# gsalzer/mythril

Measured on AMD Instinct MI355X. Metric: constraint-candidate evals/sec + % z3 queries discharged on-GPU, higher is better.
Workload: dtype u32 (256-bit as 8x32-bit limbs)

## Files before the change

mythril_amd/csrc/u256.h:

```cpp
#pragma once
#include <math.h>
#include <stdint.h>

#define PF_INL __device__ __forceinline__

#include "u256_cols.h"

namespace pf {

struct u256 {
    uint32_t l[8];
};

PF_INL u256 zero256() {
    u256 r;
#pragma unroll
    for (int i = 0; i < 8; i++) r.l[i] = 0;
    return r;
}

PF_INL u256 ones256() {
    u256 r;
#pragma unroll
    for (int i = 0; i < 8; i++) r.l[i] = 0xffffffffu;
    return r;
}

PF_INL u256 add256(const u256& a, const u256& b) {
    u256 r;
    uint32_t c = 0;
#pragma unroll
    for (int i = 0; i < 8; i++) {
        uint32_t co;
        r.l[i] = __builtin_addc(a.l[i], b.l[i], c, &co);
        c = co;
    }
    return r;
}

PF_INL u256 add256c(const u256& a, const u256& b, uint32_t* cout) {
    u256 r;
    uint32_t c = 0;
#pragma unroll
    for (int i = 0; i < 8; i++) {
        uint32_t co;
        r.l[i] = __builtin_addc(a.l[i], b.l[i], c, &co);
        c = co;
    }
    *cout = c;
    return r;
}

PF_INL u256 sub256(const u256& a, const u256& b) {
    u256 r;
    uint32_t c = 0;
#pragma unroll
    for (int i = 0; i < 8; i++) {
        uint32_t co;
        r.l[i] = __builtin_subc(a.l[i], b.l[i], c, &co);
        c = co;
    }
    return r;
}

PF_INL u256 sub256b(const u256& a, const u256& b, uint32_t* bout) {
    u256 r;
    uint32_t c = 0;
#pragma unroll
    for (int i = 0; i < 8; i++) {
        uint32_t co;
        r.l[i] = __builtin_subc(a.l[i], b.l[i], c, &co);
        c = co;
    }
    *bout = c;
    return r;
}

PF_INL uint32_t ult256(const u256& a, const u256& b) {
    uint32_t c = 0;
#pragma unroll
    for (int i = 0; i < 8; i++) {
        uint32_t co;
        (void)__builtin_subc(a.l[i], b.l[i], c, &co);
        c = co;
    }
    return c;
}

PF_INL uint32_t eq256(const u256& a, const u256& b) {
    uint32_t d = 0;
#pragma unroll
    for (int i = 0; i < 8; i++) d |= a.l[i] ^ b.l[i];
    return d == 0;
}

PF_INL uint32_t iszero256(const u256& a) {
    uint32_t d = 0;
#pragma unroll
    for (int i = 0; i < 8; i++) d |= a.l[i];
    return d == 0;
}

PF_INL u256 neg256(const u256& a) { return sub256(zero256(), a); }

PF_INL u256 not256(const u256& a) {
    u256 r;
#pragma unroll
    for (int i = 0; i < 8; i++) r.l[i] = ~a.l[i];
    return r;
}

PF_INL uint32_t lane_mask(uint32_t c) {
    uint32_t m = 0u - (uint32_t)(c != 0u);
#ifndef PF_HOST_MAC
    asm volatile("" : "+v"(m));
#endif
    return m;
}

PF_INL uint32_t zero_limb() {
    uint32_t z = 0u;
#ifndef PF_HOST_MAC
    asm("" : "+v"(z));
#endif
    return z;
}

PF_INL u256 sel256(uint32_t c, const u256& a, const u256& b) {
    const uint32_t m = lane_mask(c);
    u256 r;
#pragma unroll
    for (int i = 0; i < 8; i++) r.l[i] = (a.l[i] & m) | (b.l[i] & ~m);
    return r;
}

#ifndef PF_HOST_MAC
PF_INL uint32_t wave_max_u32(uint32_t v) {
#pragma unroll
    for (int o = 32; o >= 1; o >>= 1) v = max(v, (uint32_t)__shfl_xor((int)v, o));
    return __builtin_amdgcn_readfirstlane(v);
}
PF_INL uint64_t wave_mask(bool p) { return __builtin_amdgcn_ballot_w64(p); }
#else
PF_INL uint32_t wave_max_u32(uint32_t v) { return v; }
PF_INL uint64_t wave_mask(bool p) { return p ? 1ull : 0ull; }
#endif
PF_INL bool wave_any(uint64_t m) { return m != 0ull; }
PF_INL bool wave_none(uint64_t m) { return m == 0ull; }

PF_INL uint64_t wave_mask_ult256(const u256& a, const u256& b) {
#ifndef PF_HOST_MAC
    uint64_t m;
    uint32_t t;
    asm("v_sub_co_u32 %1, vcc, %2, %10\n\ts_nop 1\n\t"
        "v_subb_co_u32 %1, vcc, %3, %11, vcc\n\ts_nop 1\n\t"
        "v_subb_co_u32 %1, vcc, %4, %12, vcc\n\ts_nop 1\n\t"
        "v_subb_co_u32 %1, vcc, %5, %13, vcc\n\ts_nop 1\n\t"
        "v_subb_co_u32 %1, vcc, %6, %14, vcc\n\ts_nop 1\n\t"
        "v_subb_co_u32 %1, vcc, %7, %15, vcc\n\ts_nop 1\n\t"
        "v_subb_co_u32 %1, vcc, %8, %16, vcc\n\ts_nop 1\n\t"
        "v_subb_co_u32 %1, %0, %9, %17, vcc"
        : "=s"(m), "=&v"(t)
        : "v"(a.l[0]), "v"(a.l[1]), "v"(a.l[2]), "v"(a.l[3]), "v"(a.l[4]), "v"(a.l[5]), "v"(a.l[6]),
          "v"(a.l[7]), "v"(b.l[0]), "v"(b.l[1]), "v"(b.l[2]), "v"(b.l[3]), "v"(b.l[4]), "v"(b.l[5]),
          "v"(b.l[6]), "v"(b.l[7])
        : "vcc");
    return m;
#else
    return wave_mask(ult256(a, b) != 0u);
#endif
}

PF_INL uint32_t sat_u32(double x) {
#ifndef PF_HOST_MAC
    uint32_t r;
    asm("v_cvt_u32_f64 %0, %1" : "=v"(r) : "v"(x));
    return r;
#else
    return (uint32_t)fmin(x, 4294967295.0);
#endif
}

#define PF_COL_NEXT(k)                                   \
    r.l[k] = (uint32_t)acc;                              \
    acc = (acc >> 32) | ((uint64_t)hi << 32);            \
    hi = 0u;

PF_INL u256 mul256(const u256& a, const u256& b) {
    const uint32_t *x = a.l, *y = b.l;
    u256 r;
    uint64_t acc = 0;
    uint32_t hi = 0;
    col64_1(acc, x[0], y[0]);
    PF_COL_NEXT(0)
    col96_2(acc, hi, x[0], x[1], y[1], y[0]);
    PF_COL_NEXT(1)
    col96_3(acc, hi, x[0], x[1], x[2], y[2], y[1], y[0]);
    PF_COL_NEXT(2)
    col96_4(acc, hi, x[0], x[1], x[2], x[3], y[3], y[2], y[1], y[0]);
    PF_COL_NEXT(3)
    col96_5(acc, hi, x[0], x[1], x[2], x[3], x[4], y[4], y[3], y[2], y[1], y[0]);
    PF_COL_NEXT(4)
    col96_6(acc, hi, x[0], x[1], x[2], x[3], x[4], x[5], y[5], y[4], y[3], y[2], y[1], y[0]);
    PF_COL_NEXT(5)
    col64_7(acc, x[0], x[1], x[2], x[3], x[4], x[5], x[6], y[6], y[5], y[4], y[3], y[2], y[1], y[0]);
    r.l[6] = (uint32_t)acc;
    acc >>= 32;
    col64_8(acc, x[0], x[1], x[2], x[3], x[4], x[5], x[6], x[7], y[7], y[6], y[5], y[4], y[3], y[2], y[1], y[0]);
    r.l[7] = (uint32_t)acc;
    return r;
}

PF_INL u256 sqr256(const u256& a) {
    const uint32_t* x = a.l;
    u256 r;
    r.l[0] = 0u;
    uint64_t acc = 0;
    uint32_t hi = 0;
    col64_1(acc, x[0], x[1]);
    PF_COL_NEXT(1)
    col96_1(acc, hi, x[0], x[2]);
    PF_COL_NEXT(2)
    col96_2(acc, hi, x[0], x[1], x[3], x[2]);
    PF_COL_NEXT(3)
    col96_2(acc, hi, x[0], x[1], x[4], x[3]);
    PF_COL_NEXT(4)
    col96_3(acc, hi, x[0], x[1], x[2], x[5], x[4], x[3]);
    PF_COL_NEXT(5)
    col64_3(acc, x[0], x[1], x[2], x[6], x[5], x[4]);
    r.l[6] = (uint32_t)acc;
    acc >>= 32;
    col64_4(acc, x[0], x[1], x[2], x[3], x[7], x[6], x[5], x[4]);
    r.l[7] = (uint32_t)acc;
    u256 c;
#pragma unroll
    for (int i = 7; i >= 1; i--) c.l[i] = (r.l[i] << 1) | (r.l[i - 1] >> 31);
    c.l[0] = 0u;
    u256 d;
#pragma unroll
    for (int i = 0; i < 4; i++) {
        uint64_t q = 0;
        col64_1(q, x[i], x[i]);
        d.l[2 * i] = (uint32_t)q;
        d.l[2 * i + 1] = (uint32_t)(q >> 32);
    }
    return add256(c, d);
}
#undef PF_COL_NEXT

PF_INL uint32_t mul256_overflows(const u256& a, const u256& b) {
    uint32_t hi = 0;
    u256 r = zero256();
#pragma unroll
    for (int i = 0; i < 8; i++) {
        uint64_t carry = 0;
#pragma unroll
        for (int j = 0; j < 8; j++) {
            if (i + j < 8) {
                uint64_t t = (uint64_t)a.l[i] * b.l[j] + r.l[i + j] + carry;
                r.l[i + j] = (uint32_t)t;
                carry = t >> 32;
            } else {
                hi |= (a.l[i] != 0u && b.l[j] != 0u) ? 1u : 0u;
            }
        }
        hi |= (carry != 0) ? 1u : 0u;
    }
    return hi;
}

PF_INL u256 shl256(const u256& a, uint32_t s, uint32_t big) {
    u256 x = a;
    if (__builtin_expect(1, 1)) {
        uint32_t m = (s >> 7) & 1;
#pragma unroll
        for (int i = 7; i >= 0; i--) x.l[i] = m ? (i >= 4 ? x.l[i - 4] : 0u) : x.l[i];
        m = (s >> 6) & 1;
#pragma unroll
        for (int i = 7; i >= 0; i--) x.l[i] = m ? (i >= 2 ? x.l[i - 2] : 0u) : x.l[i];
        m = (s >> 5) & 1;
#pragma unroll
        for (int i = 7; i >= 0; i--) x.l[i] = m ? (i >= 1 ? x.l[i - 1] : 0u) : x.l[i];
    }
    uint32_t bs = s & 31;
    u256 r;
#pragma unroll
    for (int i = 7; i >= 1; i--) r.l[i] = bs ? ((x.l[i] << bs) | (x.l[i - 1] >> (32 - bs))) : x.l[i];
    r.l[0] = x.l[0] << bs;
    return sel256(big, zero256(), r);
}

PF_INL u256 shr256(const u256& a, uint32_t s, uint32_t f) {
    u256 x = a;
    uint32_t m = (s >> 7) & 1;
#pragma unroll
    for (int i = 0; i < 8; i++) x.l[i] = m ? (i + 4 < 8 ? x.l[i + 4] : f) : x.l[i];
    m = (s >> 6) & 1;
#pragma unroll
    for (int i = 0; i < 8; i++) x.l[i] = m ? (i + 2 < 8 ? x.l[i + 2] : f) : x.l[i];
    m = (s >> 5) & 1;
#pragma unroll
    for (int i = 0; i < 8; i++) x.l[i] = m ? (i + 1 < 8 ? x.l[i + 1] : f) : x.l[i];
    uint32_t bs = s & 31;
    u256 r;
#pragma unroll
    for (int i = 0; i < 7; i++) r.l[i] = bs ? ((x.l[i] >> bs) | (x.l[i + 1] << (32 - bs))) : x.l[i];
    r.l[7] = bs ? ((x.l[7] >> bs) | (f << (32 - bs))) : x.l[7];
    return r;
}

PF_INL uint32_t clz256(const u256& a) {
    uint32_t n = 0, done = 0;
#pragma unroll
    for (int i = 7; i >= 0; i--) {
        uint32_t z = a.l[i] ? (uint32_t)__builtin_clz(a.l[i]) : 32u;
        n += done ? 0u : z;
        done |= (a.l[i] != 0u);
    }
    return n;
}

PF_INL double rcp_f64(double x) {
#ifndef PF_HOST_MAC
    double r = __builtin_amdgcn_rcp(x);
    double e = fma(-x, r, 1.0);
    r = fma(r, e, r);
    e = fma(-x, r, 1.0);
    return fma(r, e, r);
#else
    return 1.0 / x;
#endif
}

PF_INL double to_f64(const u256& a) {
    double d = 0.0;
#pragma unroll
    for (int i = 7; i >= 0; i--) d = fma(d, 4294967296.0, (double)a.l[i]);
    return d;
}

#define PF_DIV_BIAS 0x1p-12
PF_INL void udivrem256(const u256& a, const u256& b, u256* q, u256* r) {
    const uint32_t bz = iszero256(b);
    const uint64_t m_bz = wave_mask(bz != 0u);
#ifndef PF_DIV_FORCE_GENERAL
    if (wave_none(wave_mask(true) & ~(wave_mask_ult256(a, b) | m_bz))) {
        *q = sel256(bz, ones256(), zero256());
        *r = a;
        return;
    }
    if (wave_none(wave_mask((b.l[1] | b.l[2] | b.l[3] | b.l[4] | b.l[5] | b.l[6] | b.l[7]) != 0u))) {
        const uint32_t d = bz ? 1u : b.l[0];
        const double rd = rcp_f64((double)d);
        uint32_t rem = 0;
        u256 Q;
#pragma unroll
        for (int j = 7; j >= 0; j--) {
            const uint64_t num = ((uint64_t)rem << 32) | a.l[j];
            const double dn = (double)rem * 4294967296.0 + (double)a.l[j];
            uint32_t qj = sat_u32(fma(dn, rd, 0x1p-12));
            int64_t rr = (int64_t)(num - (uint64_t)qj * d);
            const uint32_t lo = (uint32_t)(rr < 0);
            qj -= lo;
            rr += (int64_t)(d & lane_mask(lo));
            Q.l[j] = qj;
            rem = (uint32_t)rr;
        }
        u256 R = zero256();
        R.l[0] = rem;
        *q = sel256(bz, ones256(), Q);
        *r = sel256(bz, a, R);
        return;
    }
#endif
    const double rcp = rcp_f64(fmax(to_f64(b), 1.0));
#ifndef PF_DIV_FORCE_GENERAL
    const double qest = fma(to_f64(a), rcp, PF_DIV_BIAS);
    if (wave_none(wave_mask(qest >= 4294967294.0) & ~m_bz)) {
        uint32_t qh = sat_u32(qest);
        u256 R, Q = zero256();
        uint32_t carry = 0, bw = 0;
#pragma unroll
        for (int i = 0; i < 8; i++) {
            const uint64_t p = (uint64_t)qh * b.l[i] + carry;
            carry = (uint32_t)(p >> 32);
            uint32_t bo;
            R.l[i] = __builtin_subc(a.l[i], (uint32_t)p, bw, &bo);
            bw = bo;
        }
        uint32_t bo8;
        const uint32_t r8 = __builtin_subc(zero_limb(), carry, bw, &bo8);
        if (wave_any(wave_mask(r8 != 0u))) {
            const uint32_t neg = (uint32_t)(r8 != 0u);
            const uint32_t m = lane_mask(neg);
            uint32_t c = 0;
#pragma unroll
            for (int i = 0; i < 8; i++) {
                uint32_t co;
                R.l[i] = __builtin_addc(R.l[i], b.l[i] & m, c, &co);
                c = co;
            }
            qh -= neg;
        }
        Q.l[0] = qh;
        *q = sel256(bz, ones256(), Q);
        *r = R;
        return;
    }
#endif
    uint32_t u[9];
#pragma unroll
    for (int i = 0; i < 8; i++) u[i] = a.l[i];
    u256 Q = zero256();
    u[8] = zero_limb();
    uint32_t sfx[9];
    sfx[8] = 0u;
#pragma unroll
    for (int k = 7; k >= 0; k--) sfx[k] = sfx[k + 1] | b.l[k];
#pragma unroll
    for (int j = 7; j >= 0; j--) {
        const uint32_t bhigh = j >= 2 ? sfx[9 - j] : 0u;
        double dr = (double)u[7];
#pragma unroll
        for (int i = 6; i >= j; i--) dr = fma(dr, 4294967296.0, (double)u[i]);
        const double qe = fma(dr, rcp, PF_DIV_BIAS);
        if (wave_none(wave_mask(qe >= 1.0) & ~(m_bz | wave_mask(bhigh != 0u)))) continue;
        const uint32_t skip = bz | (uint32_t)(bhigh != 0u);
        uint32_t q = sat_u32(qe) & ~lane_mask(skip);
        uint64_t carry = 0;
        uint32_t borrow = 0;
#pragma unroll
        for (int i = 0; i + j <= 8; i++) {
            const uint64_t p = (uint64_t)q * (i < 8 ? b.l[i] : 0u) + carry;
            carry = p >> 32;
            uint32_t bo;
            u[j + i] = __builtin_subc(u[j + i], (uint32_t)p, borrow, &bo);
            borrow = bo;
        }
        if (wave_any(wave_mask(u[8] != 0u))) {
            const uint32_t neg = (uint32_t)(u[8] != 0u);
            const uint32_t m = 0u - neg;
            q -= neg;
            uint32_t c = 0;
#pragma unroll
            for (int i = 0; i + j <= 8; i++) {
                uint32_t co;
                u[j + i] = __builtin_addc(u[j + i], (i < 8 ? b.l[i] : 0u) & m, c, &co);
                c = co;
            }
        }
        Q.l[j] = q;
    }
    u256 R;
#pragma unroll
    for (int i = 0; i < 8; i++) R.l[i] = u[i];
    *q = sel256(bz, ones256(), Q);
    *r = R;
}

PF_INL void tbl_put(uint2* tbl, uint32_t stride, uint32_t j, const u256& v) {
#pragma unroll
    for (int p = 0; p < 4; p++) tbl[(j * 4u + p) * stride] = make_uint2(v.l[2 * p], v.l[2 * p + 1]);
}
PF_INL u256 tbl_get(const uint2* tbl, uint32_t stride, uint32_t j) {
    u256 v;
#pragma unroll
    for (int p = 0; p < 4; p++) {
        const uint2 q = tbl[(j * 4u + p) * stride];
        v.l[2 * p] = q.x;
        v.l[2 * p + 1] = q.y;
    }
    return v;
}

template <int WB = 3>
PF_INL u256 exp256(const u256& base, const u256& e, uint32_t nbits, uint2* tbl, uint32_t stride) {
    static_assert(WB >= 1 && WB <= 3, "window");
    constexpr uint32_t NT = 1u << WB;
    u256 r = zero256();
    r.l[0] = 1u;
    if (nbits == 0u) return r;
    tbl_put(tbl, stride, 0u, r);
    tbl_put(tbl, stride, 1u, base);
    if constexpr (WB == 2) {
        const u256 b2 = sqr256(base);
        tbl_put(tbl, stride, 2u, b2);
        tbl_put(tbl, stride, 3u, mul256(b2, base));
    } else {
#pragma unroll 1
        for (uint32_t j = 2; j < NT; j++) {
            const u256 f = tbl_get(tbl, stride, (j & 1u) ? j - 1u : j >> 1);
            const u256 g = (j & 1u) ? base : f;
            tbl_put(tbl, stride, j, mul256(f, g));
        }
    }
    const uint32_t nd = (nbits + WB - 1u) / WB;
    const uint32_t rest = WB * (nd - 1u);
    r = tbl_get(tbl, stride, shr256(e, rest, 0u).l[0] & (NT - 1u));
    u256 ex = shl256(e, (256u - rest) & 255u, 0u);
#pragma unroll 1
    for (uint32_t i = 1; i < nd; i++) {
#pragma unroll 1
        for (int k = 0; k < WB; k++) r = sqr256(r);
        const uint32_t d = ex.l[7] >> (32 - WB);
#pragma unroll
        for (int k = 7; k >= 1; k--) ex.l[k] = (ex.l[k] << WB) | (ex.l[k - 1] >> (32 - WB));
        ex.l[0] <<= WB;
        r = mul256(r, tbl_get(tbl, stride, d));
    }
    return r;
}

template <int WB = 2>
PF_INL u256 exp256_w32(const u256& base, uint32_t e, uint32_t nbits, uint2* tbl, uint32_t stride) {
    static_assert(WB == 2, "window");
    u256 one = zero256();
    one.l[0] = 1u;
    tbl_put(tbl, stride, 1u, base);
    const u256 b2 = sqr256(base);
    tbl_put(tbl, stride, 2u, b2);
    tbl_put(tbl, stride, 3u, mul256(b2, base));
    if (nbits == 0u) return one;
    const uint32_t nd = (nbits + WB - 1u) / WB;
    uint32_t d = (e >> (WB * (nd - 1u))) & 3u;
    u256 r = sel256((uint32_t)(d == 0u), one, tbl_get(tbl, stride, d));
#pragma unroll 1
    for (uint32_t i = nd - 1u; i-- > 0u;) {
#pragma unroll 1
        for (int k = 0; k < WB; k++) r = sqr256(r);
        d = (e >> (WB * i)) & 3u;
        r = mul256(r, sel256((uint32_t)(d == 0u), one, tbl_get(tbl, stride, d)));
    }
    return r;
}

#ifndef PF_EXP_SPLIT
#define PF_EXP_SPLIT 8
#endif
#define PF_EXP_WINDOW (PF_EXP_SPLIT <= 20 ? 2 : 3)
#define PF_EXP_TBL_ENTRIES (1 << PF_EXP_WINDOW)

PF_INL uint32_t funnel(uint32_t hi, uint32_t lo, uint32_t s) {
    return (uint32_t)((((uint64_t)hi << 32) | lo) >> s);
}

template <int L>
PF_INL void tsqr(const uint32_t* a, uint32_t* out) {
    uint32_t r[L];
#pragma unroll
    for (int i = 0; i < L; i++) r[i] = 0u;
#pragma unroll
    for (int i = 0; 2 * i + 1 < L; i++) {
        uint64_t c = 0;
#pragma unroll
        for (int j = i + 1; i + j < L; j++) {
            c = (uint64_t)a[i] * a[j] + (uint64_t)r[i + j] + (c >> 32);
            r[i + j] = (uint32_t)c;
        }
    }
#pragma unroll
    for (int i = L - 1; i >= 1; i--) r[i] = funnel(r[i], r[i - 1], 31u);
    r[0] <<= 1;
    uint32_t d[L];
#pragma unroll
    for (int i = 0; 2 * i < L; i++) {
        const uint64_t q = (uint64_t)a[i] * a[i];
        d[2 * i] = (uint32_t)q;
        if (2 * i + 1 < L) d[2 * i + 1] = (uint32_t)(q >> 32);
    }
    uint32_t c = 0;
#pragma unroll
    for (int i = 0; i < L; i++) {
        uint32_t co;
        out[i] = __builtin_addc(r[i], d[i], c, &co);
        c = co;
    }
}

template <int TL, uint32_t TM, int Q>
PF_INL void t_steps(uint32_t* t, uint32_t k0, uint32_t k1) {
    constexpr int L = TL - Q;
#pragma unroll 1
    for (uint32_t k = k0; k < k1; k++) {
        uint32_t sq[L];
        if constexpr (L == 8) {
            u256 a;
#pragma unroll
            for (int i = 0; i < 8; i++) a.l[i] = t[i];
            const u256 s = sqr256(a);
#pragma unroll
            for (int i = 0; i < 8; i++) sq[i] = s.l[i];
        } else {
            tsqr<L>(t, sq);
        }
        const uint32_t sh = 32u - (k + 1u - 32u * Q);
        uint32_t c = 0;
#pragma unroll
        for (int i = Q; i < TL; i++) {
            const uint32_t lo = i > Q ? sq[i > Q ? i - Q - 1 : 0] : 0u;
            uint32_t co;
            t[i] = __builtin_addc(t[i], funnel(sq[i - Q], lo, sh), c, &co);
            c = co;
        }
        t[TL - 1] &= TM;
    }
}


constexpr int v2c(int i) { return (i & 1) ? 0 : 1 + v2c(i >> 1); }
constexpr int v2fact(int j) { return j <= 1 ? 0 : v2c(j) + v2fact(j - 1); }
constexpr int exp_terms(int m) {
    int j = 1;
    while ((j + 1) * (m + 2) - v2fact(j + 1) < 256) j++;
    return j;
}
constexpr int prefix_val(int m, int i) { return (i - 1) * (m + 2) - v2fact(i - 1); }

struct k256 {
    uint32_t l[8];
};
constexpr k256 k_small(uint32_t v) {
    k256 r{};
    r.l[0] = v;
    return r;
}
constexpr k256 k_mul(const k256& a, const k256& b) {
    k256 r{};
    for (int i = 0; i < 8; i++) {
        uint64_t c = 0;
        for (int j = 0; i + j < 8; j++) {
            c = (uint64_t)a.l[i] * b.l[j] + r.l[i + j] + (c >> 32);
            r.l[i + j] = (uint32_t)c;
        }
    }
    return r;
}
constexpr k256 k_inv(const k256& o) {
    k256 x = o;
    for (int it = 0; it < 7; it++) {
        const k256 ox = k_mul(o, x);
        k256 two_minus{};
        uint64_t bw = 0;
        for (int i = 0; i < 8; i++) {
            const uint64_t d = (uint64_t)(i == 0 ? 2u : 0u) - ox.l[i] - bw;
            two_minus.l[i] = (uint32_t)d;
            bw = (d >> 32) & 1u;
        }
        x = k_mul(x, two_minus);
    }
    return x;
}
constexpr k256 exp_oddprod(int i, int j) {
    k256 r = k_small(1u);
    for (int k = i; k <= j; k++) r = k_mul(r, k_small((uint32_t)(k >> v2c(k))));
    return r;
}
constexpr k256 exp_addend(int i, int j, int limbs) {
    k256 r = k_mul(exp_oddprod(i, j), k_inv(exp_oddprod(1, j)));
    for (int k = limbs; k < 8; k++) r.l[k] = 0u;
    return r;
}

template <int L, int LY, uint32_t K0, uint32_t K1>
PF_INL u256 tmul_add(const u256& a, const u256& b, const k256& k) {
    if constexpr (L >= 8) {
        u256 kk;
#pragma unroll
        for (int i = 0; i < 8; i++) kk.l[i] = k.l[i];
        return add256(mul256(a, b), kk);
    } else {
        u256 r = zero256();
        tmulk<L, LY, K0, K1>(a.l, b.l, k.l, r.l);
        return r;
    }
}

template <int L>
PF_INL u256 tmul(const u256& a, const u256& b) {
    if constexpr (L >= 8)
        return mul256(a, b);
    else
        return tmul_add<L, L, 0u, 0u>(a, b, k256{});
}

template <int L>
PF_INL u256 sub_mul_small(const u256& a, const u256& b, uint32_t c) {
    u256 r = zero256();
    uint32_t carry = 0, bw = 0;
#pragma unroll
    for (int i = 0; i < L; i++) {
        const uint64_t p = (uint64_t)b.l[i] * c + carry;
        carry = (uint32_t)(p >> 32);
        uint32_t bo;
        r.l[i] = __builtin_subc(a.l[i], (uint32_t)p, bw, &bo);
        bw = bo;
    }
    return r;
}

template <int S, int L>
PF_INL u256 shl_const(const u256& a) {
    constexpr int LS = S / 32, BS = S % 32;
    u256 r = zero256();
#pragma unroll
    for (int i = LS; i < L; i++) {
        const uint32_t hi = a.l[i - LS];
        const uint32_t lo = i - LS - 1 >= 0 ? a.l[i - LS - 1 >= 0 ? i - LS - 1 : 0] : 0u;
        r.l[i] = BS ? funnel(hi, lo, 32 - BS) : hi;
    }
    return r;
}

template <int M, int I, int J>
PF_INL u256 horner(u256& g, const u256& tt) {
    constexpr int S = M + 2 - v2c(I);
    constexpr int P = 256 - prefix_val(M, I);
    constexpr int L = (P + 31) / 32;
    constexpr k256 K = exp_addend(I, J, L);
    constexpr int LY = (I == J || (P - S + 31) / 32 >= L || L == 1) ? L : L - 1;
    u256 inner = zero256();
    if constexpr (I < J) {
        inner = horner<M, I + 1, J>(g, tt);
        g = add256(g, tt);
    } else {
        constexpr k256 C = exp_addend(J + 1, J, L);
#pragma unroll
        for (int i = 0; i < L; i++) inner.l[i] = C.l[i];
    }
    return tmul_add<L, LY, K.l[0], K.l[1]>(shl_const<S, L>(g), inner, K);
}

PF_INL u256 exp256_split(const u256& base, const u256& e, uint2* tbl, uint32_t stride,
                         uint64_t* pt = nullptr) {
#if defined(PF_PROFILE_UNITS) && !defined(PF_HOST_MAC)
#define PF_EXP_STAMP(k)                                        \
    if (pt) {                                                  \
        const uint64_t t_ = __builtin_amdgcn_s_memtime();      \
        pt[k] += t_ - t_last;                                  \
        t_last = t_;                                           \
    }
    uint64_t t_last = __builtin_amdgcn_s_memtime();
#else
#define PF_EXP_STAMP(k)
    (void)pt;
#endif
    constexpr int M = PF_EXP_SPLIT;
    static_assert(M >= 8 && M <= 84, "split");
    constexpr int T = 254 - M;
    constexpr int TL = (T + 31) / 32;
    constexpr uint32_t TM = (T % 32) ? ((1u << (T % 32)) - 1u) : 0xffffffffu;
    constexpr int TB = (T + 3 + 31) / 32;
    constexpr int J = exp_terms(M);
    constexpr int WB = PF_EXP_WINDOW;
    const uint32_t odd = base.l[0] & 1u;
    const uint32_t e_big =
        (e.l[0] >= 256u) | ((e.l[1] | e.l[2] | e.l[3] | e.l[4] | e.l[5] | e.l[6] | e.l[7]) != 0u);
    u256 e0;
#pragma unroll
    for (int i = 0; i < 8; i++)
        e0.l[i] = 32 * i + 32 <= M ? e.l[i] : (32 * i < M ? e.l[i] & ((1u << (M % 32)) - 1u) : 0u);
    const uint32_t nb0 = wave_max_u32(256u - clz256(e0));
    u256 r;
    if constexpr (M <= 32 && WB == 2)
        r = exp256_w32<WB>(base, e0.l[0], nb0 < (uint32_t)M ? nb0 : (uint32_t)M, tbl, stride);
    else
        r = exp256<WB>(base, e0, nb0 < (uint32_t)M ? nb0 : (uint32_t)M, tbl, stride);
    PF_EXP_STAMP(0)
    u256 n = shr256(e, (uint32_t)M, 0u);
#pragma unroll
    for (int i = 0; i < 8; i++) n.l[i] = i < TL - 1 ? n.l[i] : (i == TL - 1 ? n.l[i] & TM : 0u);
    if (wave_any(wave_mask(odd != 0u) & ~wave_mask(iszero256(n) != 0u))) {
        tbl_put(tbl, stride, 1u, r);
        uint32_t t[TL];
        {
            uint32_t sq[TB];
            if constexpr (M <= 32 && WB == 2 && TB == 8) {
                const u256 b2 = tbl_get(tbl, stride, 2u);
#pragma unroll
                for (int i = 0; i < TB; i++) sq[i] = b2.l[i];
            } else {
                tsqr<TB>(base.l, sq);
            }
            sq[0] -= 1u;
#pragma unroll
            for (int i = 0; i < TL; i++) t[i] = funnel(i + 1 < TB ? sq[i + 1 < TB ? i + 1 : 0] : 0u, sq[i], 3u);
            t[TL - 1] &= TM;
        }
        t_steps<TL, TM, 0>(t, 1u, M < 32 ? (uint32_t)M : 32u);
        if (M > 32) t_steps<TL, TM, 1>(t, 32u, M < 64 ? (uint32_t)M : 64u);
        if (M > 64) t_steps<TL, TM, 2>(t, 64u, (uint32_t)M);
        u256 tt = zero256();
#pragma unroll
        for (int i = 0; i < TL; i++) tt.l[i] = t[i];
        PF_EXP_STAMP(1)
        const u256 nt = tmul<(256 - (M + 2) + 31) / 32>(n, tt);
        u256 g = sub_mul_small<8>(nt, tt, (uint32_t)(J - 1));
        u256 h = horner<M, 1, J>(g, tt);
        u256 one = zero256();
        one.l[0] = 1u;
        h = sel256(odd, h, one);
        r = mul256(tbl_get(tbl, stride, 1u), h);
        PF_EXP_STAMP(2)
    }
    return sel256((odd ^ 1u) & e_big, zero256(), r);
#undef PF_EXP_STAMP
}

}
```

mythril_amd/csrc/u256_cols.h:

```cpp
#pragma once
namespace pf {
#ifndef PF_HOST_MAC

PF_INL void col96_1(uint64_t& acc, uint32_t& hi, uint32_t x0, uint32_t y0) {
    uint64_t p0;
    asm("v_mad_u64_u32 %[acc], %[p0], %[x0], %[y0], %[acc]\n\ts_nop 1\n\tv_addc_co_u32_e64 %[hi], %[p0], %[hi], 0, %[p0]"
        : [acc] "+v"(acc), [hi] "+v"(hi), [p0] "=&s"(p0)
        : [x0] "v"(x0), [y0] "v"(y0));
}

PF_INL void col96_2(uint64_t& acc, uint32_t& hi, uint32_t x0, uint32_t x1, uint32_t y0, uint32_t y1) {
    uint64_t p0; uint64_t p1;
    asm("v_mad_u64_u32 %[acc], %[p0], %[x0], %[y0], %[acc]\n\tv_mad_u64_u32 %[acc], %[p1], %[x1], %[y1], %[acc]\n\ts_nop 0\n\tv_addc_co_u32_e64 %[hi], %[p0], %[hi], 0, %[p0]\n\tv_addc_co_u32_e64 %[hi], %[p1], %[hi], 0, %[p1]"
        : [acc] "+v"(acc), [hi] "+v"(hi), [p0] "=&s"(p0), [p1] "=&s"(p1)
        : [x0] "v"(x0), [x1] "v"(x1), [y0] "v"(y0), [y1] "v"(y1));
}

PF_INL void col96_3(uint64_t& acc, uint32_t& hi, uint32_t x0, uint32_t x1, uint32_t x2, uint32_t y0, uint32_t y1, uint32_t y2) {
    uint64_t p0; uint64_t p1; uint64_t p2;
    asm("v_mad_u64_u32 %[acc], %[p0], %[x0], %[y0], %[acc]\n\tv_mad_u64_u32 %[acc], %[p1], %[x1], %[y1], %[acc]\n\tv_mad_u64_u32 %[acc], %[p2], %[x2], %[y2], %[acc]\n\tv_addc_co_u32_e64 %[hi], %[p0], %[hi], 0, %[p0]\n\tv_addc_co_u32_e64 %[hi], %[p1], %[hi], 0, %[p1]\n\tv_addc_co_u32_e64 %[hi], %[p2], %[hi], 0, %[p2]"
        : [acc] "+v"(acc), [hi] "+v"(hi), [p0] "=&s"(p0), [p1] "=&s"(p1), [p2] "=&s"(p2)
        : [x0] "v"(x0), [x1] "v"(x1), [x2] "v"(x2), [y0] "v"(y0), [y1] "v"(y1), [y2] "v"(y2));
}

PF_INL void col96_4(uint64_t& acc, uint32_t& hi, uint32_t x0, uint32_t x1, uint32_t x2, uint32_t x3, uint32_t y0, uint32_t y1, uint32_t y2, uint32_t y3) {
    uint64_t p0; uint64_t p1; uint64_t p2;
    asm("v_mad_u64_u32 %[acc], %[p0], %[x0], %[y0], %[acc]\n\tv_mad_u64_u32 %[acc], %[p1], %[x1], %[y1], %[acc]\n\tv_mad_u64_u32 %[acc], %[p2], %[x2], %[y2], %[acc]\n\tv_addc_co_u32_e64 %[hi], %[p0], %[hi], 0, %[p0]\n\tv_mad_u64_u32 %[acc], %[p0], %[x3], %[y3], %[acc]\n\tv_addc_co_u32_e64 %[hi], %[p1], %[hi], 0, %[p1]\n\tv_addc_co_u32_e64 %[hi], %[p2], %[hi], 0, %[p2]\n\tv_addc_co_u32_e64 %[hi], %[p0], %[hi], 0, %[p0]"
        : [acc] "+v"(acc), [hi] "+v"(hi), [p0] "=&s"(p0), [p1] "=&s"(p1), [p2] "=&s"(p2)
        : [x0] "v"(x0), [x1] "v"(x1), [x2] "v"(x2), [x3] "v"(x3), [y0] "v"(y0), [y1] "v"(y1), [y2] "v"(y2), [y3] "v"(y3));
}

PF_INL void col96_5(uint64_t& acc, uint32_t& hi, uint32_t x0, uint32_t x1, uint32_t x2, uint32_t x3, uint32_t x4, uint32_t y0, uint32_t y1, uint32_t y2, uint32_t y3, uint32_t y4) {
    uint64_t p0; uint64_t p1; uint64_t p2;
    asm("v_mad_u64_u32 %[acc], %[p0], %[x0], %[y0], %[acc]\n\tv_mad_u64_u32 %[acc], %[p1], %[x1], %[y1], %[acc]\n\tv_mad_u64_u32 %[acc], %[p2], %[x2], %[y2], %[acc]\n\tv_addc_co_u32_e64 %[hi], %[p0], %[hi], 0, %[p0]\n\tv_mad_u64_u32 %[acc], %[p0], %[x3], %[y3], %[acc]\n\tv_addc_co_u32_e64 %[hi], %[p1], %[hi], 0, %[p1]\n\tv_mad_u64_u32 %[acc], %[p1], %[x4], %[y4], %[acc]\n\tv_addc_co_u32_e64 %[hi], %[p2], %[hi], 0, %[p2]\n\tv_addc_co_u32_e64 %[hi], %[p0], %[hi], 0, %[p0]\n\tv_addc_co_u32_e64 %[hi], %[p1], %[hi], 0, %[p1]"
        : [acc] "+v"(acc), [hi] "+v"(hi), [p0] "=&s"(p0), [p1] "=&s"(p1), [p2] "=&s"(p2)
        : [x0] "v"(x0), [x1] "v"(x1), [x2] "v"(x2), [x3] "v"(x3), [x4] "v"(x4), [y0] "v"(y0), [y1] "v"(y1), [y2] "v"(y2), [y3] "v"(y3), [y4] "v"(y4));
}

PF_INL void col96_6(uint64_t& acc, uint32_t& hi, uint32_t x0, uint32_t x1, uint32_t x2, uint32_t x3, uint32_t x4, uint32_t x5, uint32_t y0, uint32_t y1, uint32_t y2, uint32_t y3, uint32_t y4, uint32_t y5) {
    uint64_t p0; uint64_t p1; uint64_t p2;
    asm("v_mad_u64_u32 %[acc], %[p0], %[x0], %[y0], %[acc]\n\tv_mad_u64_u32 %[acc], %[p1], %[x1], %[y1], %[acc]\n\tv_mad_u64_u32 %[acc], %[p2], %[x2], %[y2], %[acc]\n\tv_addc_co_u32_e64 %[hi], %[p0], %[hi], 0, %[p0]\n\tv_mad_u64_u32 %[acc], %[p0], %[x3], %[y3], %[acc]\n\tv_addc_co_u32_e64 %[hi], %[p1], %[hi], 0, %[p1]\n\tv_mad_u64_u32 %[acc], %[p1], %[x4], %[y4], %[acc]\n\tv_addc_co_u32_e64 %[hi], %[p2], %[hi], 0, %[p2]\n\tv_mad_u64_u32 %[acc], %[p2], %[x5], %[y5], %[acc]\n\tv_addc_co_u32_e64 %[hi], %[p0], %[hi], 0, %[p0]\n\tv_addc_co_u32_e64 %[hi], %[p1], %[hi], 0, %[p1]\n\tv_addc_co_u32_e64 %[hi], %[p2], %[hi], 0, %[p2]"
        : [acc] "+v"(acc), [hi] "+v"(hi), [p0] "=&s"(p0), [p1] "=&s"(p1), [p2] "=&s"(p2)
        : [x0] "v"(x0), [x1] "v"(x1), [x2] "v"(x2), [x3] "v"(x3), [x4] "v"(x4), [x5] "v"(x5), [y0] "v"(y0), [y1] "v"(y1), [y2] "v"(y2), [y3] "v"(y3), [y4] "v"(y4), [y5] "v"(y5));
}

PF_INL void col64_1(uint64_t& acc, uint32_t x0, uint32_t y0) {
    uint64_t p;
    asm("v_mad_u64_u32 %[acc], %[p], %[x0], %[y0], %[acc]"
        : [acc] "+v"(acc), [p] "=&s"(p)
        : [x0] "v"(x0), [y0] "v"(y0));
}

PF_INL void col64_2(uint64_t& acc, uint32_t x0, uint32_t x1, uint32_t y0, uint32_t y1) {
    uint64_t p;
    asm("v_mad_u64_u32 %[acc], %[p], %[x0], %[y0], %[acc]\n\tv_mad_u64_u32 %[acc], %[p], %[x1], %[y1], %[acc]"
        : [acc] "+v"(acc), [p] "=&s"(p)
        : [x0] "v"(x0), [x1] "v"(x1), [y0] "v"(y0), [y1] "v"(y1));
}

PF_INL void col64_3(uint64_t& acc, uint32_t x0, uint32_t x1, uint32_t x2, uint32_t y0, uint32_t y1, uint32_t y2) {
    uint64_t p;
    asm("v_mad_u64_u32 %[acc], %[p], %[x0], %[y0], %[acc]\n\tv_mad_u64_u32 %[acc], %[p], %[x1], %[y1], %[acc]\n\tv_mad_u64_u32 %[acc], %[p], %[x2], %[y2], %[acc]"
        : [acc] "+v"(acc), [p] "=&s"(p)
        : [x0] "v"(x0), [x1] "v"(x1), [x2] "v"(x2), [y0] "v"(y0), [y1] "v"(y1), [y2] "v"(y2));
}

PF_INL void col64_4(uint64_t& acc, uint32_t x0, uint32_t x1, uint32_t x2, uint32_t x3, uint32_t y0, uint32_t y1, uint32_t y2, uint32_t y3) {
    uint64_t p;
    asm("v_mad_u64_u32 %[acc], %[p], %[x0], %[y0], %[acc]\n\tv_mad_u64_u32 %[acc], %[p], %[x1], %[y1], %[acc]\n\tv_mad_u64_u32 %[acc], %[p], %[x2], %[y2], %[acc]\n\tv_mad_u64_u32 %[acc], %[p], %[x3], %[y3], %[acc]"
        : [acc] "+v"(acc), [p] "=&s"(p)
        : [x0] "v"(x0), [x1] "v"(x1), [x2] "v"(x2), [x3] "v"(x3), [y0] "v"(y0), [y1] "v"(y1), [y2] "v"(y2), [y3] "v"(y3));
}

PF_INL void col64_5(uint64_t& acc, uint32_t x0, uint32_t x1, uint32_t x2, uint32_t x3, uint32_t x4, uint32_t y0, uint32_t y1, uint32_t y2, uint32_t y3, uint32_t y4) {
    uint64_t p;
    asm("v_mad_u64_u32 %[acc], %[p], %[x0], %[y0], %[acc]\n\tv_mad_u64_u32 %[acc], %[p], %[x1], %[y1], %[acc]\n\tv_mad_u64_u32 %[acc], %[p], %[x2], %[y2], %[acc]\n\tv_mad_u64_u32 %[acc], %[p], %[x3], %[y3], %[acc]\n\tv_mad_u64_u32 %[acc], %[p], %[x4], %[y4], %[acc]"
        : [acc] "+v"(acc), [p] "=&s"(p)
        : [x0] "v"(x0), [x1] "v"(x1), [x2] "v"(x2), [x3] "v"(x3), [x4] "v"(x4), [y0] "v"(y0), [y1] "v"(y1), [y2] "v"(y2), [y3] "v"(y3), [y4] "v"(y4));
}

PF_INL void col64_6(uint64_t& acc, uint32_t x0, uint32_t x1, uint32_t x2, uint32_t x3, uint32_t x4, uint32_t x5, uint32_t y0, uint32_t y1, uint32_t y2, uint32_t y3, uint32_t y4, uint32_t y5) {
    uint64_t p;
    asm("v_mad_u64_u32 %[acc], %[p], %[x0], %[y0], %[acc]\n\tv_mad_u64_u32 %[acc], %[p], %[x1], %[y1], %[acc]\n\tv_mad_u64_u32 %[acc], %[p], %[x2], %[y2], %[acc]\n\tv_mad_u64_u32 %[acc], %[p], %[x3], %[y3], %[acc]\n\tv_mad_u64_u32 %[acc], %[p], %[x4], %[y4], %[acc]\n\tv_mad_u64_u32 %[acc], %[p], %[x5], %[y5], %[acc]"
        : [acc] "+v"(acc), [p] "=&s"(p)
        : [x0] "v"(x0), [x1] "v"(x1), [x2] "v"(x2), [x3] "v"(x3), [x4] "v"(x4), [x5] "v"(x5), [y0] "v"(y0), [y1] "v"(y1), [y2] "v"(y2), [y3] "v"(y3), [y4] "v"(y4), [y5] "v"(y5));
}

PF_INL void col64_7(uint64_t& acc, uint32_t x0, uint32_t x1, uint32_t x2, uint32_t x3, uint32_t x4, uint32_t x5, uint32_t x6, uint32_t y0, uint32_t y1, uint32_t y2, uint32_t y3, uint32_t y4, uint32_t y5, uint32_t y6) {
    uint64_t p;
    asm("v_mad_u64_u32 %[acc], %[p], %[x0], %[y0], %[acc]\n\tv_mad_u64_u32 %[acc], %[p], %[x1], %[y1], %[acc]\n\tv_mad_u64_u32 %[acc], %[p], %[x2], %[y2], %[acc]\n\tv_mad_u64_u32 %[acc], %[p], %[x3], %[y3], %[acc]\n\tv_mad_u64_u32 %[acc], %[p], %[x4], %[y4], %[acc]\n\tv_mad_u64_u32 %[acc], %[p], %[x5], %[y5], %[acc]\n\tv_mad_u64_u32 %[acc], %[p], %[x6], %[y6], %[acc]"
        : [acc] "+v"(acc), [p] "=&s"(p)
        : [x0] "v"(x0), [x1] "v"(x1), [x2] "v"(x2), [x3] "v"(x3), [x4] "v"(x4), [x5] "v"(x5), [x6] "v"(x6), [y0] "v"(y0), [y1] "v"(y1), [y2] "v"(y2), [y3] "v"(y3), [y4] "v"(y4), [y5] "v"(y5), [y6] "v"(y6));
}

PF_INL void col64_8(uint64_t& acc, uint32_t x0, uint32_t x1, uint32_t x2, uint32_t x3, uint32_t x4, uint32_t x5, uint32_t x6, uint32_t x7, uint32_t y0, uint32_t y1, uint32_t y2, uint32_t y3, uint32_t y4, uint32_t y5, uint32_t y6, uint32_t y7) {
    uint64_t p;
    asm("v_mad_u64_u32 %[acc], %[p], %[x0], %[y0], %[acc]\n\tv_mad_u64_u32 %[acc], %[p], %[x1], %[y1], %[acc]\n\tv_mad_u64_u32 %[acc], %[p], %[x2], %[y2], %[acc]\n\tv_mad_u64_u32 %[acc], %[p], %[x3], %[y3], %[acc]\n\tv_mad_u64_u32 %[acc], %[p], %[x4], %[y4], %[acc]\n\tv_mad_u64_u32 %[acc], %[p], %[x5], %[y5], %[acc]\n\tv_mad_u64_u32 %[acc], %[p], %[x6], %[y6], %[acc]\n\tv_mad_u64_u32 %[acc], %[p], %[x7], %[y7], %[acc]"
        : [acc] "+v"(acc), [p] "=&s"(p)
        : [x0] "v"(x0), [x1] "v"(x1), [x2] "v"(x2), [x3] "v"(x3), [x4] "v"(x4), [x5] "v"(x5), [x6] "v"(x6), [x7] "v"(x7), [y0] "v"(y0), [y1] "v"(y1), [y2] "v"(y2), [y3] "v"(y3), [y4] "v"(y4), [y5] "v"(y5), [y6] "v"(y6), [y7] "v"(y7));
}

#else

PF_INL void col96_1(uint64_t& acc, uint32_t& hi, uint32_t x0, uint32_t y0) {
    { unsigned __int128 t = (unsigned __int128)x0 * y0 + acc; acc = (uint64_t)t; hi += (uint32_t)(t >> 64); }
}

PF_INL void col96_2(uint64_t& acc, uint32_t& hi, uint32_t x0, uint32_t x1, uint32_t y0, uint32_t y1) {
    { unsigned __int128 t = (unsigned __int128)x0 * y0 + acc; acc = (uint64_t)t; hi += (uint32_t)(t >> 64); }
    { unsigned __int128 t = (unsigned __int128)x1 * y1 + acc; acc = (uint64_t)t; hi += (uint32_t)(t >> 64); }
}

PF_INL void col96_3(uint64_t& acc, uint32_t& hi, uint32_t x0, uint32_t x1, uint32_t x2, uint32_t y0, uint32_t y1, uint32_t y2) {
    { unsigned __int128 t = (unsigned __int128)x0 * y0 + acc; acc = (uint64_t)t; hi += (uint32_t)(t >> 64); }
    { unsigned __int128 t = (unsigned __int128)x1 * y1 + acc; acc = (uint64_t)t; hi += (uint32_t)(t >> 64); }
    { unsigned __int128 t = (unsigned __int128)x2 * y2 + acc; acc = (uint64_t)t; hi += (uint32_t)(t >> 64); }
}

PF_INL void col96_4(uint64_t& acc, uint32_t& hi, uint32_t x0, uint32_t x1, uint32_t x2, uint32_t x3, uint32_t y0, uint32_t y1, uint32_t y2, uint32_t y3) {
    { unsigned __int128 t = (unsigned __int128)x0 * y0 + acc; acc = (uint64_t)t; hi += (uint32_t)(t >> 64); }
    { unsigned __int128 t = (unsigned __int128)x1 * y1 + acc; acc = (uint64_t)t; hi += (uint32_t)(t >> 64); }
    { unsigned __int128 t = (unsigned __int128)x2 * y2 + acc; acc = (uint64_t)t; hi += (uint32_t)(t >> 64); }
    { unsigned __int128 t = (unsigned __int128)x3 * y3 + acc; acc = (uint64_t)t; hi += (uint32_t)(t >> 64); }
}

PF_INL void col96_5(uint64_t& acc, uint32_t& hi, uint32_t x0, uint32_t x1, uint32_t x2, uint32_t x3, uint32_t x4, uint32_t y0, uint32_t y1, uint32_t y2, uint32_t y3, uint32_t y4) {
    { unsigned __int128 t = (unsigned __int128)x0 * y0 + acc; acc = (uint64_t)t; hi += (uint32_t)(t >> 64); }
    { unsigned __int128 t = (unsigned __int128)x1 * y1 + acc; acc = (uint64_t)t; hi += (uint32_t)(t >> 64); }
    { unsigned __int128 t = (unsigned __int128)x2 * y2 + acc; acc = (uint64_t)t; hi += (uint32_t)(t >> 64); }
    { unsigned __int128 t = (unsigned __int128)x3 * y3 + acc; acc = (uint64_t)t; hi += (uint32_t)(t >> 64); }
    { unsigned __int128 t = (unsigned __int128)x4 * y4 + acc; acc = (uint64_t)t; hi += (uint32_t)(t >> 64); }
}

PF_INL void col96_6(uint64_t& acc, uint32_t& hi, uint32_t x0, uint32_t x1, uint32_t x2, uint32_t x3, uint32_t x4, uint32_t x5, uint32_t y0, uint32_t y1, uint32_t y2, uint32_t y3, uint32_t y4, uint32_t y5) {
    { unsigned __int128 t = (unsigned __int128)x0 * y0 + acc; acc = (uint64_t)t; hi += (uint32_t)(t >> 64); }
    { unsigned __int128 t = (unsigned __int128)x1 * y1 + acc; acc = (uint64_t)t; hi += (uint32_t)(t >> 64); }
    { unsigned __int128 t = (unsigned __int128)x2 * y2 + acc; acc = (uint64_t)t; hi += (uint32_t)(t >> 64); }
    { unsigned __int128 t = (unsigned __int128)x3 * y3 + acc; acc = (uint64_t)t; hi += (uint32_t)(t >> 64); }
    { unsigned __int128 t = (unsigned __int128)x4 * y4 + acc; acc = (uint64_t)t; hi += (uint32_t)(t >> 64); }
    { unsigned __int128 t = (unsigned __int128)x5 * y5 + acc; acc = (uint64_t)t; hi += (uint32_t)(t >> 64); }
}

PF_INL void col64_1(uint64_t& acc, uint32_t x0, uint32_t y0) {
    acc += (uint64_t)x0 * y0;
}

PF_INL void col64_2(uint64_t& acc, uint32_t x0, uint32_t x1, uint32_t y0, uint32_t y1) {
    acc += (uint64_t)x0 * y0;
    acc += (uint64_t)x1 * y1;
}

PF_INL void col64_3(uint64_t& acc, uint32_t x0, uint32_t x1, uint32_t x2, uint32_t y0, uint32_t y1, uint32_t y2) {
    acc += (uint64_t)x0 * y0;
    acc += (uint64_t)x1 * y1;
    acc += (uint64_t)x2 * y2;
}

PF_INL void col64_4(uint64_t& acc, uint32_t x0, uint32_t x1, uint32_t x2, uint32_t x3, uint32_t y0, uint32_t y1, uint32_t y2, uint32_t y3) {
    acc += (uint64_t)x0 * y0;
    acc += (uint64_t)x1 * y1;
    acc += (uint64_t)x2 * y2;
    acc += (uint64_t)x3 * y3;
}

PF_INL void col64_5(uint64_t& acc, uint32_t x0, uint32_t x1, uint32_t x2, uint32_t x3, uint32_t x4, uint32_t y0, uint32_t y1, uint32_t y2, uint32_t y3, uint32_t y4) {
    acc += (uint64_t)x0 * y0;
    acc += (uint64_t)x1 * y1;
    acc += (uint64_t)x2 * y2;
    acc += (uint64_t)x3 * y3;
    acc += (uint64_t)x4 * y4;
}

PF_INL void col64_6(uint64_t& acc, uint32_t x0, uint32_t x1, uint32_t x2, uint32_t x3, uint32_t x4, uint32_t x5, uint32_t y0, uint32_t y1, uint32_t y2, uint32_t y3, uint32_t y4, uint32_t y5) {
    acc += (uint64_t)x0 * y0;
    acc += (uint64_t)x1 * y1;
    acc += (uint64_t)x2 * y2;
    acc += (uint64_t)x3 * y3;
    acc += (uint64_t)x4 * y4;
    acc += (uint64_t)x5 * y5;
}

PF_INL void col64_7(uint64_t& acc, uint32_t x0, uint32_t x1, uint32_t x2, uint32_t x3, uint32_t x4, uint32_t x5, uint32_t x6, uint32_t y0, uint32_t y1, uint32_t y2, uint32_t y3, uint32_t y4, uint32_t y5, uint32_t y6) {
    acc += (uint64_t)x0 * y0;
    acc += (uint64_t)x1 * y1;
    acc += (uint64_t)x2 * y2;
    acc += (uint64_t)x3 * y3;
    acc += (uint64_t)x4 * y4;
    acc += (uint64_t)x5 * y5;
    acc += (uint64_t)x6 * y6;
}

PF_INL void col64_8(uint64_t& acc, uint32_t x0, uint32_t x1, uint32_t x2, uint32_t x3, uint32_t x4, uint32_t x5, uint32_t x6, uint32_t x7, uint32_t y0, uint32_t y1, uint32_t y2, uint32_t y3, uint32_t y4, uint32_t y5, uint32_t y6, uint32_t y7) {
    acc += (uint64_t)x0 * y0;
    acc += (uint64_t)x1 * y1;
    acc += (uint64_t)x2 * y2;
    acc += (uint64_t)x3 * y3;
    acc += (uint64_t)x4 * y4;
    acc += (uint64_t)x5 * y5;
    acc += (uint64_t)x6 * y6;
    acc += (uint64_t)x7 * y7;
}

#endif

template <uint32_t K0, uint32_t K1>
PF_INL uint64_t acc_const() {
#ifndef PF_HOST_MAC
    if constexpr (K0 != 0u || K1 != 0u) {
        uint32_t lo, up;
        asm volatile("v_mov_b32 %0, %2\n\tv_mov_b32 %1, %3" : "=v"(lo), "=v"(up) : "i"(K0), "i"(K1));
        return (uint64_t)lo | ((uint64_t)up << 32);
    }
#endif
    return (uint64_t)K0 | ((uint64_t)K1 << 32);
}

template <uint32_t K0, uint32_t K1>
PF_INL void tmulk_1_1(const uint32_t* x, const uint32_t* y, const uint32_t* k, uint32_t* r) {
    uint64_t acc = acc_const<K0, 0u>();
    uint32_t hi = 0u;
    col64_1(acc, x[0], y[0]);
    r[0] = (uint32_t)acc;
    (void)hi;
}

template <uint32_t K0, uint32_t K1>
PF_INL void tmulk_2_1(const uint32_t* x, const uint32_t* y, const uint32_t* k, uint32_t* r) {
    uint64_t acc = acc_const<K0, K1>();
    uint32_t hi = 0u;
    col64_1(acc, x[0], y[0]);
    r[0] = (uint32_t)acc;
    acc >>= 32;
    col64_1(acc, x[1], y[0]);
    r[1] = (uint32_t)acc;
    (void)hi;
}

template <uint32_t K0, uint32_t K1>
PF_INL void tmulk_2_2(const uint32_t* x, const uint32_t* y, const uint32_t* k, uint32_t* r) {
    uint64_t acc = acc_const<K0, K1>();
    uint32_t hi = 0u;
    col64_1(acc, x[0], y[0]);
    r[0] = (uint32_t)acc;
    acc >>= 32;
    col64_2(acc, x[0], x[1], y[1], y[0]);
    r[1] = (uint32_t)acc;
    (void)hi;
}

template <uint32_t K0, uint32_t K1>
PF_INL void tmulk_3_2(const uint32_t* x, const uint32_t* y, const uint32_t* k, uint32_t* r) {
    uint64_t acc = acc_const<K0, K1>();
    uint32_t hi = 0u;
    col96_1(acc, hi, x[0], y[0]);
    r[0] = (uint32_t)acc;
    { const uint64_t t = (uint64_t)hi + k[2]; acc = (acc >> 32) | (t << 32); hi = (uint32_t)(t >> 32); }
    col64_2(acc, x[0], x[1], y[1], y[0]);
    r[1] = (uint32_t)acc;
    acc >>= 32;
    col64_2(acc, x[1], x[2], y[1], y[0]);
    r[2] = (uint32_t)acc;
    (void)hi;
}

template <uint32_t K0, uint32_t K1>
PF_INL void tmulk_3_3(const uint32_t* x, const uint32_t* y, const uint32_t* k, uint32_t* r) {
    uint64_t acc = acc_const<K0, K1>();
    uint32_t hi = 0u;
    col96_1(acc, hi, x[0], y[0]);
    r[0] = (uint32_t)acc;
    { const uint64_t t = (uint64_t)hi + k[2]; acc = (acc >> 32) | (t << 32); hi = (uint32_t)(t >> 32); }
    col64_2(acc, x[0], x[1], y[1], y[0]);
    r[1] = (uint32_t)acc;
    acc >>= 32;
    col64_3(acc, x[0], x[1], x[2], y[2], y[1], y[0]);
    r[2] = (uint32_t)acc;
    (void)hi;
}

template <uint32_t K0, uint32_t K1>
PF_INL void tmulk_4_3(const uint32_t* x, const uint32_t* y, const uint32_t* k, uint32_t* r) {
    uint64_t acc = acc_const<K0, K1>();
    uint32_t hi = 0u;
    col96_1(acc, hi, x[0], y[0]);
    r[0] = (uint32_t)acc;
    { const uint64_t t = (uint64_t)hi + k[2]; acc = (acc >> 32) | (t << 32); hi = (uint32_t)(t >> 32); }
    col96_2(acc, hi, x[0], x[1], y[1], y[0]);
    r[1] = (uint32_t)acc;
    { const uint64_t t = (uint64_t)hi + k[3]; acc = (acc >> 32) | (t << 32); hi = (uint32_t)(t >> 32); }
    col64_3(acc, x[0], x[1], x[2], y[2], y[1], y[0]);
    r[2] = (uint32_t)acc;
    acc >>= 32;
    col64_3(acc, x[1], x[2], x[3], y[2], y[1], y[0]);
    r[3] = (uint32_t)acc;
    (void)hi;
}

template <uint32_t K0, uint32_t K1>
PF_INL void tmulk_4_4(const uint32_t* x, const uint32_t* y, const uint32_t* k, uint32_t* r) {
    uint64_t acc = acc_const<K0, K1>();
    uint32_t hi = 0u;
    col96_1(acc, hi, x[0], y[0]);
    r[0] = (uint32_t)acc;
    { const uint64_t t = (uint64_t)hi + k[2]; acc = (acc >> 32) | (t << 32); hi = (uint32_t)(t >> 32); }
    col96_2(acc, hi, x[0], x[1], y[1], y[0]);
    r[1] = (uint32_t)acc;
    { const uint64_t t = (uint64_t)hi + k[3]; acc = (acc >> 32) | (t << 32); hi = (uint32_t)(t >> 32); }
    col64_3(acc, x[0], x[1], x[2], y[2], y[1], y[0]);
    r[2] = (uint32_t)acc;
    acc >>= 32;
    col64_4(acc, x[0], x[1], x[2], x[3], y[3], y[2], y[1], y[0]);
    r[3] = (uint32_t)acc;
    (void)hi;
}

template <uint32_t K0, uint32_t K1>
PF_INL void tmulk_5_4(const uint32_t* x, const uint32_t* y, const uint32_t* k, uint32_t* r) {
    uint64_t acc = acc_const<K0, K1>();
    uint32_t hi = 0u;
    col96_1(acc, hi, x[0], y[0]);
    r[0] = (uint32_t)acc;
    { const uint64_t t = (uint64_t)hi + k[2]; acc = (acc >> 32) | (t << 32); hi = (uint32_t)(t >> 32); }
    col96_2(acc, hi, x[0], x[1], y[1], y[0]);
    r[1] = (uint32_t)acc;
    { const uint64_t t = (uint64_t)hi + k[3]; acc = (acc >> 32) | (t << 32); hi = (uint32_t)(t >> 32); }
    col96_3(acc, hi, x[0], x[1], x[2], y[2], y[1], y[0]);
    r[2] = (uint32_t)acc;
    { const uint64_t t = (uint64_t)hi + k[4]; acc = (acc >> 32) | (t << 32); hi = (uint32_t)(t >> 32); }
    col64_4(acc, x[0], x[1], x[2], x[3], y[3], y[2], y[1], y[0]);
    r[3] = (uint32_t)acc;
    acc >>= 32;
    col64_4(acc, x[1], x[2], x[3], x[4], y[3], y[2], y[1], y[0]);
    r[4] = (uint32_t)acc;
    (void)hi;
}

template <uint32_t K0, uint32_t K1>
PF_INL void tmulk_5_5(const uint32_t* x, const uint32_t* y, const uint32_t* k, uint32_t* r) {
    uint64_t acc = acc_const<K0, K1>();
    uint32_t hi = 0u;
    col96_1(acc, hi, x[0], y[0]);
    r[0] = (uint32_t)acc;
    { const uint64_t t = (uint64_t)hi + k[2]; acc = (acc >> 32) | (t << 32); hi = (uint32_t)(t >> 32); }
    col96_2(acc, hi, x[0], x[1], y[1], y[0]);
    r[1] = (uint32_t)acc;
    { const uint64_t t = (uint64_t)hi + k[3]; acc = (acc >> 32) | (t << 32); hi = (uint32_t)(t >> 32); }
    col96_3(acc, hi, x[0], x[1], x[2], y[2], y[1], y[0]);
    r[2] = (uint32_t)acc;
    { const uint64_t t = (uint64_t)hi + k[4]; acc = (acc >> 32) | (t << 32); hi = (uint32_t)(t >> 32); }
    col64_4(acc, x[0], x[1], x[2], x[3], y[3], y[2], y[1], y[0]);
    r[3] = (uint32_t)acc;
    acc >>= 32;
    col64_5(acc, x[0], x[1], x[2], x[3], x[4], y[4], y[3], y[2], y[1], y[0]);
    r[4] = (uint32_t)acc;
    (void)hi;
}

template <uint32_t K0, uint32_t K1>
PF_INL void tmulk_6_5(const uint32_t* x, const uint32_t* y, const uint32_t* k, uint32_t* r) {
    uint64_t acc = acc_const<K0, K1>();
    uint32_t hi = 0u;
    col96_1(acc, hi, x[0], y[0]);
    r[0] = (uint32_t)acc;
    { const uint64_t t = (uint64_t)hi + k[2]; acc = (acc >> 32) | (t << 32); hi = (uint32_t)(t >> 32); }
    col96_2(acc, hi, x[0], x[1], y[1], y[0]);
    r[1] = (uint32_t)acc;
    { const uint64_t t = (uint64_t)hi + k[3]; acc = (acc >> 32) | (t << 32); hi = (uint32_t)(t >> 32); }
    col96_3(acc, hi, x[0], x[1], x[2], y[2], y[1], y[0]);
    r[2] = (uint32_t)acc;
    { const uint64_t t = (uint64_t)hi + k[4]; acc = (acc >> 32) | (t << 32); hi = (uint32_t)(t >> 32); }
    col96_4(acc, hi, x[0], x[1], x[2], x[3], y[3], y[2], y[1], y[0]);
    r[3] = (uint32_t)acc;
    { const uint64_t t = (uint64_t)hi + k[5]; acc = (acc >> 32) | (t << 32); hi = (uint32_t)(t >> 32); }
    col64_5(acc, x[0], x[1], x[2], x[3], x[4], y[4], y[3], y[2], y[1], y[0]);
    r[4] = (uint32_t)acc;
    acc >>= 32;
    col64_5(acc, x[1], x[2], x[3], x[4], x[5], y[4], y[3], y[2], y[1], y[0]);
    r[5] = (uint32_t)acc;
    (void)hi;
}

template <uint32_t K0, uint32_t K1>
PF_INL void tmulk_6_6(const uint32_t* x, const uint32_t* y, const uint32_t* k, uint32_t* r) {
    uint64_t acc = acc_const<K0, K1>();
    uint32_t hi = 0u;
    col96_1(acc, hi, x[0], y[0]);
    r[0] = (uint32_t)acc;
    { const uint64_t t = (uint64_t)hi + k[2]; acc = (acc >> 32) | (t << 32); hi = (uint32_t)(t >> 32); }
    col96_2(acc, hi, x[0], x[1], y[1], y[0]);
    r[1] = (uint32_t)acc;
    { const uint64_t t = (uint64_t)hi + k[3]; acc = (acc >> 32) | (t << 32); hi = (uint32_t)(t >> 32); }
    col96_3(acc, hi, x[0], x[1], x[2], y[2], y[1], y[0]);
    r[2] = (uint32_t)acc;
    { const uint64_t t = (uint64_t)hi + k[4]; acc = (acc >> 32) | (t << 32); hi = (uint32_t)(t >> 32); }
    col96_4(acc, hi, x[0], x[1], x[2], x[3], y[3], y[2], y[1], y[0]);
    r[3] = (uint32_t)acc;
    { const uint64_t t = (uint64_t)hi + k[5]; acc = (acc >> 32) | (t << 32); hi = (uint32_t)(t >> 32); }
    col64_5(acc, x[0], x[1], x[2], x[3], x[4], y[4], y[3], y[2], y[1], y[0]);
    r[4] = (uint32_t)acc;
    acc >>= 32;
    col64_6(acc, x[0], x[1], x[2], x[3], x[4], x[5], y[5], y[4], y[3], y[2], y[1], y[0]);
    r[5] = (uint32_t)acc;
    (void)hi;
}

template <uint32_t K0, uint32_t K1>
PF_INL void tmulk_7_6(const uint32_t* x, const uint32_t* y, const uint32_t* k, uint32_t* r) {
    uint64_t acc = acc_const<K0, K1>();
    uint32_t hi = 0u;
    col96_1(acc, hi, x[0], y[0]);
    r[0] = (uint32_t)acc;
    { const uint64_t t = (uint64_t)hi + k[2]; acc = (acc >> 32) | (t << 32); hi = (uint32_t)(t >> 32); }
    col96_2(acc, hi, x[0], x[1], y[1], y[0]);
    r[1] = (uint32_t)acc;
    { const uint64_t t = (uint64_t)hi + k[3]; acc = (acc >> 32) | (t << 32); hi = (uint32_t)(t >> 32); }
    col96_3(acc, hi, x[0], x[1], x[2], y[2], y[1], y[0]);
    r[2] = (uint32_t)acc;
    { const uint64_t t = (uint64_t)hi + k[4]; acc = (acc >> 32) | (t << 32); hi = (uint32_t)(t >> 32); }
    col96_4(acc, hi, x[0], x[1], x[2], x[3], y[3], y[2], y[1], y[0]);
    r[3] = (uint32_t)acc;
    { const uint64_t t = (uint64_t)hi + k[5]; acc = (acc >> 32) | (t << 32); hi = (uint32_t)(t >> 32); }
    col96_5(acc, hi, x[0], x[1], x[2], x[3], x[4], y[4], y[3], y[2], y[1], y[0]);
    r[4] = (uint32_t)acc;
    { const uint64_t t = (uint64_t)hi + k[6]; acc = (acc >> 32) | (t << 32); hi = (uint32_t)(t >> 32); }
    col64_6(acc, x[0], x[1], x[2], x[3], x[4], x[5], y[5], y[4], y[3], y[2], y[1], y[0]);
    r[5] = (uint32_t)acc;
    acc >>= 32;
    col64_6(acc, x[1], x[2], x[3], x[4], x[5], x[6], y[5], y[4], y[3], y[2], y[1], y[0]);
    r[6] = (uint32_t)acc;
    (void)hi;
}

template <uint32_t K0, uint32_t K1>
PF_INL void tmulk_7_7(const uint32_t* x, const uint32_t* y, const uint32_t* k, uint32_t* r) {
    uint64_t acc = acc_const<K0, K1>();
    uint32_t hi = 0u;
    col96_1(acc, hi, x[0], y[0]);
    r[0] = (uint32_t)acc;
    { const uint64_t t = (uint64_t)hi + k[2]; acc = (acc >> 32) | (t << 32); hi = (uint32_t)(t >> 32); }
    col96_2(acc, hi, x[0], x[1], y[1], y[0]);
    r[1] = (uint32_t)acc;
    { const uint64_t t = (uint64_t)hi + k[3]; acc = (acc >> 32) | (t << 32); hi = (uint32_t)(t >> 32); }
    col96_3(acc, hi, x[0], x[1], x[2], y[2], y[1], y[0]);
    r[2] = (uint32_t)acc;
    { const uint64_t t = (uint64_t)hi + k[4]; acc = (acc >> 32) | (t << 32); hi = (uint32_t)(t >> 32); }
    col96_4(acc, hi, x[0], x[1], x[2], x[3], y[3], y[2], y[1], y[0]);
    r[3] = (uint32_t)acc;
    { const uint64_t t = (uint64_t)hi + k[5]; acc = (acc >> 32) | (t << 32); hi = (uint32_t)(t >> 32); }
    col96_5(acc, hi, x[0], x[1], x[2], x[3], x[4], y[4], y[3], y[2], y[1], y[0]);
    r[4] = (uint32_t)acc;
    { const uint64_t t = (uint64_t)hi + k[6]; acc = (acc >> 32) | (t << 32); hi = (uint32_t)(t >> 32); }
    col64_6(acc, x[0], x[1], x[2], x[3], x[4], x[5], y[5], y[4], y[3], y[2], y[1], y[0]);
    r[5] = (uint32_t)acc;
    acc >>= 32;
    col64_7(acc, x[0], x[1], x[2], x[3], x[4], x[5], x[6], y[6], y[5], y[4], y[3], y[2], y[1], y[0]);
    r[6] = (uint32_t)acc;
    (void)hi;
}

template <int L, int LY, uint32_t K0, uint32_t K1>
PF_INL void tmulk(const uint32_t* x, const uint32_t* y, const uint32_t* k, uint32_t* r) {
    static_assert(L >= 1 && L <= 7 && (LY == L || LY == L - 1) && LY >= 1, "shape");
    if constexpr (L == 1 && LY == 1) tmulk_1_1<K0, K1>(x, y, k, r);
    if constexpr (L == 2 && LY == 1) tmulk_2_1<K0, K1>(x, y, k, r);
    if constexpr (L == 2 && LY == 2) tmulk_2_2<K0, K1>(x, y, k, r);
    if constexpr (L == 3 && LY == 2) tmulk_3_2<K0, K1>(x, y, k, r);
    if constexpr (L == 3 && LY == 3) tmulk_3_3<K0, K1>(x, y, k, r);
    if constexpr (L == 4 && LY == 3) tmulk_4_3<K0, K1>(x, y, k, r);
    if constexpr (L == 4 && LY == 4) tmulk_4_4<K0, K1>(x, y, k, r);
    if constexpr (L == 5 && LY == 4) tmulk_5_4<K0, K1>(x, y, k, r);
    if constexpr (L == 5 && LY == 5) tmulk_5_5<K0, K1>(x, y, k, r);
    if constexpr (L == 6 && LY == 5) tmulk_6_5<K0, K1>(x, y, k, r);
    if constexpr (L == 6 && LY == 6) tmulk_6_6<K0, K1>(x, y, k, r);
    if constexpr (L == 7 && LY == 6) tmulk_7_6<K0, K1>(x, y, k, r);
    if constexpr (L == 7 && LY == 7) tmulk_7_7<K0, K1>(x, y, k, r);
}

}
```

Baseline: 7.361 billion.

## Fold addend limbs as template constants and zero hi in carry asm

The truncated multiply-add kernels now take all addend limbs as compile-time template parameters and add them directly into the 32-bit carry word, dropping the 64-bit add-with-carry per column. Zero-addend shapes get dedicated plain multiply variants. The column asm now seeds the hi carry from the constant 0 instead of reading and then resetting a register. Separately, the windowed small-exponent path skips building the power table when the exponent has at most one bit, and the series-needed test is hoisted so b^2 is only computed when the later stage uses it. Static asserts guard the assumption that each addend limb plus accumulated carries fits in 32 bits.

After: 7.449 billion (median of 6 runs). +1.2%, better.

```diff
diff --git a/mythril_amd/csrc/u256.h b/mythril_amd/csrc/u256.h
--- a/mythril_amd/csrc/u256.h
+++ b/mythril_amd/csrc/u256.h
@@ -183,8 +183,7 @@
 
 #define PF_COL_NEXT(k)                                   \
     r.l[k] = (uint32_t)acc;                              \
-    acc = (acc >> 32) | ((uint64_t)hi << 32);            \
-    hi = 0u;
+    acc = (acc >> 32) | ((uint64_t)hi << 32);
 
 PF_INL u256 mul256(const u256& a, const u256& b) {
     const uint32_t *x = a.l, *y = b.l;
@@ -512,15 +511,20 @@
 }
 
 template <int WB = 2>
-PF_INL u256 exp256_w32(const u256& base, uint32_t e, uint32_t nbits, uint2* tbl, uint32_t stride) {
+PF_INL u256 exp256_w32(const u256& base, uint32_t e, uint32_t nbits, bool want_b2, uint2* tbl, uint32_t stride) {
     static_assert(WB == 2, "window");
     u256 one = zero256();
     one.l[0] = 1u;
-    tbl_put(tbl, stride, 1u, base);
-    const u256 b2 = sqr256(base);
-    tbl_put(tbl, stride, 2u, b2);
-    tbl_put(tbl, stride, 3u, mul256(b2, base));
-    if (nbits == 0u) return one;
+    const bool loop = nbits > 1u;
+    if (loop || want_b2) {
+        const u256 b2 = sqr256(base);
+        tbl_put(tbl, stride, 2u, b2);
+        if (loop) {
+            tbl_put(tbl, stride, 1u, base);
+            tbl_put(tbl, stride, 3u, mul256(b2, base));
+        }
+    }
+    if (!loop) return sel256((uint32_t)(e == 0u), one, base);
     const uint32_t nd = (nbits + WB - 1u) / WB;
     uint32_t d = (e >> (WB * (nd - 1u))) & 3u;
     u256 r = sel256((uint32_t)(d == 0u), one, tbl_get(tbl, stride, d));
@@ -661,7 +665,7 @@
     return r;
 }
 
-template <int L, int LY, uint32_t K0, uint32_t K1>
+template <int L, int LY, uint32_t K0, uint32_t K1, uint32_t K2, uint32_t K3, uint32_t K4, uint32_t K5, uint32_t K6>
 PF_INL u256 tmul_add(const u256& a, const u256& b, const k256& k) {
     if constexpr (L >= 8) {
         u256 kk;
@@ -670,7 +674,7 @@
         return add256(mul256(a, b), kk);
     } else {
         u256 r = zero256();
-        tmulk<L, LY, K0, K1>(a.l, b.l, k.l, r.l);
+        tmulk<L, LY, K0, K1, K2, K3, K4, K5, K6>(a.l, b.l, r.l);
         return r;
     }
 }
@@ -680,7 +684,7 @@
     if constexpr (L >= 8)
         return mul256(a, b);
     else
-        return tmul_add<L, L, 0u, 0u>(a, b, k256{});
+        return tmul_add<L, L, 0u, 0u, 0u, 0u, 0u, 0u, 0u>(a, b, k256{});
 }
 
 template <int L>
@@ -727,7 +731,7 @@
 #pragma unroll
         for (int i = 0; i < L; i++) inner.l[i] = C.l[i];
     }
-    return tmul_add<L, LY, K.l[0], K.l[1]>(shl_const<S, L>(g), inner, K);
+    return tmul_add<L, LY, K.l[0], K.l[1], K.l[2], K.l[3], K.l[4], K.l[5], K.l[6]>(shl_const<S, L>(g), inner, K);
 }
 
 PF_INL u256 exp256_split(const u256& base, const u256& e, uint2* tbl, uint32_t stride,
@@ -760,16 +764,17 @@
     for (int i = 0; i < 8; i++)
         e0.l[i] = 32 * i + 32 <= M ? e.l[i] : (32 * i < M ? e.l[i] & ((1u << (M % 32)) - 1u) : 0u);
     const uint32_t nb0 = wave_max_u32(256u - clz256(e0));
+    u256 n = shr256(e, (uint32_t)M, 0u);
+#pragma unroll
+    for (int i = 0; i < 8; i++) n.l[i] = i < TL - 1 ? n.l[i] : (i == TL - 1 ? n.l[i] & TM : 0u);
+    const bool series = wave_any(wave_mask(odd != 0u) & ~wave_mask(iszero256(n) != 0u));
     u256 r;
     if constexpr (M <= 32 && WB == 2)
-        r = exp256_w32<WB>(base, e0.l[0], nb0 < (uint32_t)M ? nb0 : (uint32_t)M, tbl, stride);
+        r = exp256_w32<WB>(base, e0.l[0], nb0 < (uint32_t)M ? nb0 : (uint32_t)M, series && TB == 8, tbl, stride);
     else
         r = exp256<WB>(base, e0, nb0 < (uint32_t)M ? nb0 : (uint32_t)M, tbl, stride);
     PF_EXP_STAMP(0)
-    u256 n = shr256(e, (uint32_t)M, 0u);
-#pragma unroll
-    for (int i = 0; i < 8; i++) n.l[i] = i < TL - 1 ? n.l[i] : (i == TL - 1 ? n.l[i] & TM : 0u);
-    if (wave_any(wave_mask(odd != 0u) & ~wave_mask(iszero256(n) != 0u))) {
+    if (series) {
         tbl_put(tbl, stride, 1u, r);
         uint32_t t[TL];
         {
diff --git a/mythril_amd/csrc/u256_cols.h b/mythril_amd/csrc/u256_cols.h
--- a/mythril_amd/csrc/u256_cols.h
+++ b/mythril_amd/csrc/u256_cols.h
@@ -4,43 +4,43 @@
 
 PF_INL void col96_1(uint64_t& acc, uint32_t& hi, uint32_t x0, uint32_t y0) {
     uint64_t p0;
-    asm("v_mad_u64_u32 %[acc], %[p0], %[x0], %[y0], %[acc]\n\ts_nop 1\n\tv_addc_co_u32_e64 %[hi], %[p0], %[hi], 0, %[p0]"
-        : [acc] "+v"(acc), [hi] "+v"(hi), [p0] "=&s"(p0)
+    asm("v_mad_u64_u32 %[acc], %[p0], %[x0], %[y0], %[acc]\n\ts_nop 1\n\tv_addc_co_u32_e64 %[hi], %[p0], 0, 0, %[p0]"
+        : [acc] "+v"(acc), [hi] "=&v"(hi), [p0] "=&s"(p0)
         : [x0] "v"(x0), [y0] "v"(y0));
 }
 
 PF_INL void col96_2(uint64_t& acc, uint32_t& hi, uint32_t x0, uint32_t x1, uint32_t y0, uint32_t y1) {
     uint64_t p0; uint64_t p1;
-    asm("v_mad_u64_u32 %[acc], %[p0], %[x0], %[y0], %[acc]\n\tv_mad_u64_u32 %[acc], %[p1], %[x1], %[y1], %[acc]\n\ts_nop 0\n\tv_addc_co_u32_e64 %[hi], %[p0], %[hi], 0, %[p0]\n\tv_addc_co_u32_e64 %[hi], %[p1], %[hi], 0, %[p1]"
-        : [acc] "+v"(acc), [hi] "+v"(hi), [p0] "=&s"(p0), [p1] "=&s"(p1)
+    asm("v_mad_u64_u32 %[acc], %[p0], %[x0], %[y0], %[acc]\n\tv_mad_u64_u32 %[acc], %[p1], %[x1], %[y1], %[acc]\n\ts_nop 0\n\tv_addc_co_u32_e64 %[hi], %[p0], 0, 0, %[p0]\n\tv_addc_co_u32_e64 %[hi], %[p1], %[hi], 0, %[p1]"
+        : [acc] "+v"(acc), [hi] "=&v"(hi), [p0] "=&s"(p0), [p1] "=&s"(p1)
         : [x0] "v"(x0), [x1] "v"(x1), [y0] "v"(y0), [y1] "v"(y1));
 }
 
 PF_INL void col96_3(uint64_t& acc, uint32_t& hi, uint32_t x0, uint32_t x1, uint32_t x2, uint32_t y0, uint32_t y1, uint32_t y2) {
     uint64_t p0; uint64_t p1; uint64_t p2;
-    asm("v_mad_u64_u32 %[acc], %[p0], %[x0], %[y0], %[acc]\n\tv_mad_u64_u32 %[acc], %[p1], %[x1], %[y1], %[acc]\n\tv_mad_u64_u32 %[acc], %[p2], %[x2], %[y2], %[acc]\n\tv_addc_co_u32_e64 %[hi], %[p0], %[hi], 0, %[p0]\n\tv_addc_co_u32_e64 %[hi], %[p1], %[hi], 0, %[p1]\n\tv_addc_co_u32_e64 %[hi], %[p2], %[hi], 0, %[p2]"
-        : [acc] "+v"(acc), [hi] "+v"(hi), [p0] "=&s"(p0), [p1] "=&s"(p1), [p2] "=&s"(p2)
+    asm("v_mad_u64_u32 %[acc], %[p0], %[x0], %[y0], %[acc]\n\tv_mad_u64_u32 %[acc], %[p1], %[x1], %[y1], %[acc]\n\tv_mad_u64_u32 %[acc], %[p2], %[x2], %[y2], %[acc]\n\tv_addc_co_u32_e64 %[hi], %[p0], 0, 0, %[p0]\n\tv_addc_co_u32_e64 %[hi], %[p1], %[hi], 0, %[p1]\n\tv_addc_co_u32_e64 %[hi], %[p2], %[hi], 0, %[p2]"
+        : [acc] "+v"(acc), [hi] "=&v"(hi), [p0] "=&s"(p0), [p1] "=&s"(p1), [p2] "=&s"(p2)
         : [x0] "v"(x0), [x1] "v"(x1), [x2] "v"(x2), [y0] "v"(y0), [y1] "v"(y1), [y2] "v"(y2));
 }
 
 PF_INL void col96_4(uint64_t& acc, uint32_t& hi, uint32_t x0, uint32_t x1, uint32_t x2, uint32_t x3, uint32_t y0, uint32_t y1, uint32_t y2, uint32_t y3) {
     uint64_t p0; uint64_t p1; uint64_t p2;
-    asm("v_mad_u64_u32 %[acc], %[p0], %[x0], %[y0], %[acc]\n\tv_mad_u64_u32 %[acc], %[p1], %[x1], %[y1], %[acc]\n\tv_mad_u64_u32 %[acc], %[p2], %[x2], %[y2], %[acc]\n\tv_addc_co_u32_e64 %[hi], %[p0], %[hi], 0, %[p0]\n\tv_mad_u64_u32 %[acc], %[p0], %[x3], %[y3], %[acc]\n\tv_addc_co_u32_e64 %[hi], %[p1], %[hi], 0, %[p1]\n\tv_addc_co_u32_e64 %[hi], %[p2], %[hi], 0, %[p2]\n\tv_addc_co_u32_e64 %[hi], %[p0], %[hi], 0, %[p0]"
-        : [acc] "+v"(acc), [hi] "+v"(hi), [p0] "=&s"(p0), [p1] "=&s"(p1), [p2] "=&s"(p2)
+    asm("v_mad_u64_u32 %[acc], %[p0], %[x0], %[y0], %[acc]\n\tv_mad_u64_u32 %[acc], %[p1], %[x1], %[y1], %[acc]\n\tv_mad_u64_u32 %[acc], %[p2], %[x2], %[y2], %[acc]\n\tv_addc_co_u32_e64 %[hi], %[p0], 0, 0, %[p0]\n\tv_mad_u64_u32 %[acc], %[p0], %[x3], %[y3], %[acc]\n\tv_addc_co_u32_e64 %[hi], %[p1], %[hi], 0, %[p1]\n\tv_addc_co_u32_e64 %[hi], %[p2], %[hi], 0, %[p2]\n\tv_addc_co_u32_e64 %[hi], %[p0], %[hi], 0, %[p0]"
+        : [acc] "+v"(acc), [hi] "=&v"(hi), [p0] "=&s"(p0), [p1] "=&s"(p1), [p2] "=&s"(p2)
         : [x0] "v"(x0), [x1] "v"(x1), [x2] "v"(x2), [x3] "v"(x3), [y0] "v"(y0), [y1] "v"(y1), [y2] "v"(y2), [y3] "v"(y3));
 }
 
 PF_INL void col96_5(uint64_t& acc, uint32_t& hi, uint32_t x0, uint32_t x1, uint32_t x2, uint32_t x3, uint32_t x4, uint32_t y0, uint32_t y1, uint32_t y2, uint32_t y3, uint32_t y4) {
     uint64_t p0; uint64_t p1; uint64_t p2;
-    asm("v_mad_u64_u32 %[acc], %[p0], %[x0], %[y0], %[acc]\n\tv_mad_u64_u32 %[acc], %[p1], %[x1], %[y1], %[acc]\n\tv_mad_u64_u32 %[acc], %[p2], %[x2], %[y2], %[acc]\n\tv_addc_co_u32_e64 %[hi], %[p0], %[hi], 0, %[p0]\n\tv_mad_u64_u32 %[acc], %[p0], %[x3], %[y3], %[acc]\n\tv_addc_co_u32_e64 %[hi], %[p1], %[hi], 0, %[p1]\n\tv_mad_u64_u32 %[acc], %[p1], %[x4], %[y4], %[acc]\n\tv_addc_co_u32_e64 %[hi], %[p2], %[hi], 0, %[p2]\n\tv_addc_co_u32_e64 %[hi], %[p0], %[hi], 0, %[p0]\n\tv_addc_co_u32_e64 %[hi], %[p1], %[hi], 0, %[p1]"
-        : [acc] "+v"(acc), [hi] "+v"(hi), [p0] "=&s"(p0), [p1] "=&s"(p1), [p2] "=&s"(p2)
+    asm("v_mad_u64_u32 %[acc], %[p0], %[x0], %[y0], %[acc]\n\tv_mad_u64_u32 %[acc], %[p1], %[x1], %[y1], %[acc]\n\tv_mad_u64_u32 %[acc], %[p2], %[x2], %[y2], %[acc]\n\tv_addc_co_u32_e64 %[hi], %[p0], 0, 0, %[p0]\n\tv_mad_u64_u32 %[acc], %[p0], %[x3], %[y3], %[acc]\n\tv_addc_co_u32_e64 %[hi], %[p1], %[hi], 0, %[p1]\n\tv_mad_u64_u32 %[acc], %[p1], %[x4], %[y4], %[acc]\n\tv_addc_co_u32_e64 %[hi], %[p2], %[hi], 0, %[p2]\n\tv_addc_co_u32_e64 %[hi], %[p0], %[hi], 0, %[p0]\n\tv_addc_co_u32_e64 %[hi], %[p1], %[hi], 0, %[p1]"
+        : [acc] "+v"(acc), [hi] "=&v"(hi), [p0] "=&s"(p0), [p1] "=&s"(p1), [p2] "=&s"(p2)
         : [x0] "v"(x0), [x1] "v"(x1), [x2] "v"(x2), [x3] "v"(x3), [x4] "v"(x4), [y0] "v"(y0), [y1] "v"(y1), [y2] "v"(y2), [y3] "v"(y3), [y4] "v"(y4));
 }
 
 PF_INL void col96_6(uint64_t& acc, uint32_t& hi, uint32_t x0, uint32_t x1, uint32_t x2, uint32_t x3, uint32_t x4, uint32_t x5, uint32_t y0, uint32_t y1, uint32_t y2, uint32_t y3, uint32_t y4, uint32_t y5) {
     uint64_t p0; uint64_t p1; uint64_t p2;
-    asm("v_mad_u64_u32 %[acc], %[p0], %[x0], %[y0], %[acc]\n\tv_mad_u64_u32 %[acc], %[p1], %[x1], %[y1], %[acc]\n\tv_mad_u64_u32 %[acc], %[p2], %[x2], %[y2], %[acc]\n\tv_addc_co_u32_e64 %[hi], %[p0], %[hi], 0, %[p0]\n\tv_mad_u64_u32 %[acc], %[p0], %[x3], %[y3], %[acc]\n\tv_addc_co_u32_e64 %[hi], %[p1], %[hi], 0, %[p1]\n\tv_mad_u64_u32 %[acc], %[p1], %[x4], %[y4], %[acc]\n\tv_addc_co_u32_e64 %[hi], %[p2], %[hi], 0, %[p2]\n\tv_mad_u64_u32 %[acc], %[p2], %[x5], %[y5], %[acc]\n\tv_addc_co_u32_e64 %[hi], %[p0], %[hi], 0, %[p0]\n\tv_addc_co_u32_e64 %[hi], %[p1], %[hi], 0, %[p1]\n\tv_addc_co_u32_e64 %[hi], %[p2], %[hi], 0, %[p2]"
-        : [acc] "+v"(acc), [hi] "+v"(hi), [p0] "=&s"(p0), [p1] "=&s"(p1), [p2] "=&s"(p2)
+    asm("v_mad_u64_u32 %[acc], %[p0], %[x0], %[y0], %[acc]\n\tv_mad_u64_u32 %[acc], %[p1], %[x1], %[y1], %[acc]\n\tv_mad_u64_u32 %[acc], %[p2], %[x2], %[y2], %[acc]\n\tv_addc_co_u32_e64 %[hi], %[p0], 0, 0, %[p0]\n\tv_mad_u64_u32 %[acc], %[p0], %[x3], %[y3], %[acc]\n\tv_addc_co_u32_e64 %[hi], %[p1], %[hi], 0, %[p1]\n\tv_mad_u64_u32 %[acc], %[p1], %[x4], %[y4], %[acc]\n\tv_addc_co_u32_e64 %[hi], %[p2], %[hi], 0, %[p2]\n\tv_mad_u64_u32 %[acc], %[p2], %[x5], %[y5], %[acc]\n\tv_addc_co_u32_e64 %[hi], %[p0], %[hi], 0, %[p0]\n\tv_addc_co_u32_e64 %[hi], %[p1], %[hi], 0, %[p1]\n\tv_addc_co_u32_e64 %[hi], %[p2], %[hi], 0, %[p2]"
+        : [acc] "+v"(acc), [hi] "=&v"(hi), [p0] "=&s"(p0), [p1] "=&s"(p1), [p2] "=&s"(p2)
         : [x0] "v"(x0), [x1] "v"(x1), [x2] "v"(x2), [x3] "v"(x3), [x4] "v"(x4), [x5] "v"(x5), [y0] "v"(y0), [y1] "v"(y1), [y2] "v"(y2), [y3] "v"(y3), [y4] "v"(y4), [y5] "v"(y5));
 }
 
@@ -103,21 +103,25 @@
 #else
 
 PF_INL void col96_1(uint64_t& acc, uint32_t& hi, uint32_t x0, uint32_t y0) {
+    hi = 0u;
     { unsigned __int128 t = (unsigned __int128)x0 * y0 + acc; acc = (uint64_t)t; hi += (uint32_t)(t >> 64); }
 }
 
 PF_INL void col96_2(uint64_t& acc, uint32_t& hi, uint32_t x0, uint32_t x1, uint32_t y0, uint32_t y1) {
+    hi = 0u;
     { unsigned __int128 t = (unsigned __int128)x0 * y0 + acc; acc = (uint64_t)t; hi += (uint32_t)(t >> 64); }
     { unsigned __int128 t = (unsigned __int128)x1 * y1 + acc; acc = (uint64_t)t; hi += (uint32_t)(t >> 64); }
 }
 
 PF_INL void col96_3(uint64_t& acc, uint32_t& hi, uint32_t x0, uint32_t x1, uint32_t x2, uint32_t y0, uint32_t y1, uint32_t y2) {
+    hi = 0u;
     { unsigned __int128 t = (unsigned __int128)x0 * y0 + acc; acc = (uint64_t)t; hi += (uint32_t)(t >> 64); }
     { unsigned __int128 t = (unsigned __int128)x1 * y1 + acc; acc = (uint64_t)t; hi += (uint32_t)(t >> 64); }
     { unsigned __int128 t = (unsigned __int128)x2 * y2 + acc; acc = (uint64_t)t; hi += (uint32_t)(t >> 64); }
 }
 
 PF_INL void col96_4(uint64_t& acc, uint32_t& hi, uint32_t x0, uint32_t x1, uint32_t x2, uint32_t x3, uint32_t y0, uint32_t y1, uint32_t y2, uint32_t y3) {
+    hi = 0u;
     { unsigned __int128 t = (unsigned __int128)x0 * y0 + acc; acc = (uint64_t)t; hi += (uint32_t)(t >> 64); }
     { unsigned __int128 t = (unsigned __int128)x1 * y1 + acc; acc = (uint64_t)t; hi += (uint32_t)(t >> 64); }
     { unsigned __int128 t = (unsigned __int128)x2 * y2 + acc; acc = (uint64_t)t; hi += (uint32_t)(t >> 64); }
@@ -125,6 +129,7 @@
 }
 
 PF_INL void col96_5(uint64_t& acc, uint32_t& hi, uint32_t x0, uint32_t x1, uint32_t x2, uint32_t x3, uint32_t x4, uint32_t y0, uint32_t y1, uint32_t y2, uint32_t y3, uint32_t y4) {
+    hi = 0u;
     { unsigned __int128 t = (unsigned __int128)x0 * y0 + acc; acc = (uint64_t)t; hi += (uint32_t)(t >> 64); }
     { unsigned __int128 t = (unsigned __int128)x1 * y1 + acc; acc = (uint64_t)t; hi += (uint32_t)(t >> 64); }
     { unsigned __int128 t = (unsigned __int128)x2 * y2 + acc; acc = (uint64_t)t; hi += (uint32_t)(t >> 64); }
@@ -133,6 +138,7 @@
 }
 
 PF_INL void col96_6(uint64_t& acc, uint32_t& hi, uint32_t x0, uint32_t x1, uint32_t x2, uint32_t x3, uint32_t x4, uint32_t x5, uint32_t y0, uint32_t y1, uint32_t y2, uint32_t y3, uint32_t y4, uint32_t y5) {
+    hi = 0u;
     { unsigned __int128 t = (unsigned __int128)x0 * y0 + acc; acc = (uint64_t)t; hi += (uint32_t)(t >> 64); }
     { unsigned __int128 t = (unsigned __int128)x1 * y1 + acc; acc = (uint64_t)t; hi += (uint32_t)(t >> 64); }
     { unsigned __int128 t = (unsigned __int128)x2 * y2 + acc; acc = (uint64_t)t; hi += (uint32_t)(t >> 64); }
@@ -215,265 +221,537 @@
     return (uint64_t)K0 | ((uint64_t)K1 << 32);
 }
 
+template <uint32_t K0>
+PF_INL void tmulk_1_1(const uint32_t* x, const uint32_t* y, uint32_t* r) {
+    uint64_t acc = acc_const<K0, 0u>();
+    col64_1(acc, x[0], y[0]);
+    r[0] = (uint32_t)acc;
+}
+
+PF_INL void tmul_1_1(const uint32_t* x, const uint32_t* y, uint32_t* r) {
+    uint64_t acc = 0;
+    col64_1(acc, x[0], y[0]);
+    r[0] = (uint32_t)acc;
+}
+
 template <uint32_t K0, uint32_t K1>
-PF_INL void tmulk_1_1(const uint32_t* x, const uint32_t* y, const uint32_t* k, uint32_t* r) {
-    uint64_t acc = acc_const<K0, 0u>();
-    uint32_t hi = 0u;
+PF_INL void tmulk_2_1(const uint32_t* x, const uint32_t* y, uint32_t* r) {
+    uint64_t acc = acc_const<K0, K1>();
     col64_1(acc, x[0], y[0]);
     r[0] = (uint32_t)acc;
-    (void)hi;
+    acc >>= 32;
+    col64_1(acc, x[1], y[0]);
+    r[1] = (uint32_t)acc;
+}
+
+PF_INL void tmul_2_1(const uint32_t* x, const uint32_t* y, uint32_t* r) {
+    uint64_t acc = 0;
+    col64_1(acc, x[0], y[0]);
+    r[0] = (uint32_t)acc;
+    acc >>= 32;
+    col64_1(acc, x[1], y[0]);
+    r[1] = (uint32_t)acc;
 }
 
 template <uint32_t K0, uint32_t K1>
-PF_INL void tmulk_2_1(const uint32_t* x, const uint32_t* y, const uint32_t* k, uint32_t* r) {
-    uint64_t acc = acc_const<K0, K1>();
-    uint32_t hi = 0u;
+PF_INL void tmulk_2_2(const uint32_t* x, const uint32_t* y, uint32_t* r) {
+    uint64_t acc = acc_const<K0, K1>();
     col64_1(acc, x[0], y[0]);
     r[0] = (uint32_t)acc;
     acc >>= 32;
-    col64_1(acc, x[1], y[0]);
-    r[1] = (uint32_t)acc;
-    (void)hi;
-}
-
-template <uint32_t K0, uint32_t K1>
-PF_INL void tmulk_2_2(const uint32_t* x, const uint32_t* y, const uint32_t* k, uint32_t* r) {
-    uint64_t acc = acc_const<K0, K1>();
-    uint32_t hi = 0u;
+    col64_2(acc, x[0], x[1], y[1], y[0]);
+    r[1] = (uint32_t)acc;
+}
+
+PF_INL void tmul_2_2(const uint32_t* x, const uint32_t* y, uint32_t* r) {
+    uint64_t acc = 0;
     col64_1(acc, x[0], y[0]);
     r[0] = (uint32_t)acc;
     acc >>= 32;
     col64_2(acc, x[0], x[1], y[1], y[0]);
     r[1] = (uint32_t)acc;
-    (void)hi;
-}
-
-template <uint32_t K0, uint32_t K1>
-PF_INL void tmulk_3_2(const uint32_t* x, const uint32_t* y, const uint32_t* k, uint32_t* r) {
-    uint64_t acc = acc_const<K0, K1>();
-    uint32_t hi = 0u;
-    col96_1(acc, hi, x[0], y[0]);
-    r[0] = (uint32_t)acc;
-    { const uint64_t t = (uint64_t)hi + k[2]; acc = (acc >> 32) | (t << 32); hi = (uint32_t)(t >> 32); }
+}
+
+template <uint32_t K0, uint32_t K1, uint32_t K2>
+PF_INL void tmulk_3_2(const uint32_t* x, const uint32_t* y, uint32_t* r) {
+    uint64_t acc = acc_const<K0, K1>();
+    uint32_t hi;
+    col96_1(acc, hi, x[0], y[0]);
+    r[0] = (uint32_t)acc;
+    static_assert(K2 <= 0xFFFFFFFFu - 1u, "addend limb + 1 carries must fit 32 bits");
+    hi += K2;
+    acc = (acc >> 32) | ((uint64_t)hi << 32);
     col64_2(acc, x[0], x[1], y[1], y[0]);
     r[1] = (uint32_t)acc;
     acc >>= 32;
     col64_2(acc, x[1], x[2], y[1], y[0]);
     r[2] = (uint32_t)acc;
-    (void)hi;
-}
-
-template <uint32_t K0, uint32_t K1>
-PF_INL void tmulk_3_3(const uint32_t* x, const uint32_t* y, const uint32_t* k, uint32_t* r) {
-    uint64_t acc = acc_const<K0, K1>();
-    uint32_t hi = 0u;
-    col96_1(acc, hi, x[0], y[0]);
-    r[0] = (uint32_t)acc;
-    { const uint64_t t = (uint64_t)hi + k[2]; acc = (acc >> 32) | (t << 32); hi = (uint32_t)(t >> 32); }
+}
+
+PF_INL void tmul_3_2(const uint32_t* x, const uint32_t* y, uint32_t* r) {
+    uint64_t acc = 0;
+    uint32_t hi;
+    col96_1(acc, hi, x[0], y[0]);
+    r[0] = (uint32_t)acc;
+    acc = (acc >> 32) | ((uint64_t)hi << 32);
     col64_2(acc, x[0], x[1], y[1], y[0]);
     r[1] = (uint32_t)acc;
     acc >>= 32;
+    col64_2(acc, x[1], x[2], y[1], y[0]);
+    r[2] = (uint32_t)acc;
+}
+
+template <uint32_t K0, uint32_t K1, uint32_t K2>
+PF_INL void tmulk_3_3(const uint32_t* x, const uint32_t* y, uint32_t* r) {
+    uint64_t acc = acc_const<K0, K1>();
+    uint32_t hi;
+    col96_1(acc, hi, x[0], y[0]);
+    r[0] = (uint32_t)acc;
+    static_assert(K2 <= 0xFFFFFFFFu - 1u, "addend limb + 1 carries must fit 32 bits");
+    hi += K2;
+    acc = (acc >> 32) | ((uint64_t)hi << 32);
+    col64_2(acc, x[0], x[1], y[1], y[0]);
+    r[1] = (uint32_t)acc;
+    acc >>= 32;
     col64_3(acc, x[0], x[1], x[2], y[2], y[1], y[0]);
     r[2] = (uint32_t)acc;
-    (void)hi;
-}
-
-template <uint32_t K0, uint32_t K1>
-PF_INL void tmulk_4_3(const uint32_t* x, const uint32_t* y, const uint32_t* k, uint32_t* r) {
-    uint64_t acc = acc_const<K0, K1>();
-    uint32_t hi = 0u;
-    col96_1(acc, hi, x[0], y[0]);
-    r[0] = (uint32_t)acc;
-    { const uint64_t t = (uint64_t)hi + k[2]; acc = (acc >> 32) | (t << 32); hi = (uint32_t)(t >> 32); }
-    col96_2(acc, hi, x[0], x[1], y[1], y[0]);
-    r[1] = (uint32_t)acc;
-    { const uint64_t t = (uint64_t)hi + k[3]; acc = (acc >> 32) | (t << 32); hi = (uint32_t)(t >> 32); }
+}
+
+PF_INL void tmul_3_3(const uint32_t* x, const uint32_t* y, uint32_t* r) {
+    uint64_t acc = 0;
+    uint32_t hi;
+    col96_1(acc, hi, x[0], y[0]);
+    r[0] = (uint32_t)acc;
+    acc = (acc >> 32) | ((uint64_t)hi << 32);
+    col64_2(acc, x[0], x[1], y[1], y[0]);
+    r[1] = (uint32_t)acc;
+    acc >>= 32;
     col64_3(acc, x[0], x[1], x[2], y[2], y[1], y[0]);
     r[2] = (uint32_t)acc;
+}
+
+template <uint32_t K0, uint32_t K1, uint32_t K2, uint32_t K3>
+PF_INL void tmulk_4_3(const uint32_t* x, const uint32_t* y, uint32_t* r) {
+    uint64_t acc = acc_const<K0, K1>();
+    uint32_t hi;
+    col96_1(acc, hi, x[0], y[0]);
+    r[0] = (uint32_t)acc;
+    static_assert(K2 <= 0xFFFFFFFFu - 1u, "addend limb + 1 carries must fit 32 bits");
+    hi += K2;
+    acc = (acc >> 32) | ((uint64_t)hi << 32);
+    col96_2(acc, hi, x[0], x[1], y[1], y[0]);
+    r[1] = (uint32_t)acc;
+    static_assert(K3 <= 0xFFFFFFFFu - 2u, "addend limb + 2 carries must fit 32 bits");
+    hi += K3;
+    acc = (acc >> 32) | ((uint64_t)hi << 32);
+    col64_3(acc, x[0], x[1], x[2], y[2], y[1], y[0]);
+    r[2] = (uint32_t)acc;
     acc >>= 32;
     col64_3(acc, x[1], x[2], x[3], y[2], y[1], y[0]);
     r[3] = (uint32_t)acc;
-    (void)hi;
-}
-
-template <uint32_t K0, uint32_t K1>
-PF_INL void tmulk_4_4(const uint32_t* x, const uint32_t* y, const uint32_t* k, uint32_t* r) {
-    uint64_t acc = acc_const<K0, K1>();
-    uint32_t hi = 0u;
-    col96_1(acc, hi, x[0], y[0]);
-    r[0] = (uint32_t)acc;
-    { const uint64_t t = (uint64_t)hi + k[2]; acc = (acc >> 32) | (t << 32); hi = (uint32_t)(t >> 32); }
-    col96_2(acc, hi, x[0], x[1], y[1], y[0]);
-    r[1] = (uint32_t)acc;
-    { const uint64_t t = (uint64_t)hi + k[3]; acc = (acc >> 32) | (t << 32); hi = (uint32_t)(t >> 32); }
+}
+
+PF_INL void tmul_4_3(const uint32_t* x, const uint32_t* y, uint32_t* r) {
+    uint64_t acc = 0;
+    uint32_t hi;
+    col96_1(acc, hi, x[0], y[0]);
+    r[0] = (uint32_t)acc;
+    acc = (acc >> 32) | ((uint64_t)hi << 32);
+    col96_2(acc, hi, x[0], x[1], y[1], y[0]);
+    r[1] = (uint32_t)acc;
+    acc = (acc >> 32) | ((uint64_t)hi << 32);
     col64_3(acc, x[0], x[1], x[2], y[2], y[1], y[0]);
     r[2] = (uint32_t)acc;
     acc >>= 32;
+    col64_3(acc, x[1], x[2], x[3], y[2], y[1], y[0]);
+    r[3] = (uint32_t)acc;
+}
+
+template <uint32_t K0, uint32_t K1, uint32_t K2, uint32_t K3>
+PF_INL void tmulk_4_4(const uint32_t* x, const uint32_t* y, uint32_t* r) {
+    uint64_t acc = acc_const<K0, K1>();
+    uint32_t hi;
+    col96_1(acc, hi, x[0], y[0]);
+    r[0] = (uint32_t)acc;
+    static_assert(K2 <= 0xFFFFFFFFu - 1u, "addend limb + 1 carries must fit 32 bits");
+    hi += K2;
+    acc = (acc >> 32) | ((uint64_t)hi << 32);
+    col96_2(acc, hi, x[0], x[1], y[1], y[0]);
+    r[1] = (uint32_t)acc;
+    static_assert(K3 <= 0xFFFFFFFFu - 2u, "addend limb + 2 carries must fit 32 bits");
+    hi += K3;
+    acc = (acc >> 32) | ((uint64_t)hi << 32);
+    col64_3(acc, x[0], x[1], x[2], y[2], y[1], y[0]);
+    r[2] = (uint32_t)acc;
+    acc >>= 32;
     col64_4(acc, x[0], x[1], x[2], x[3], y[3], y[2], y[1], y[0]);
     r[3] = (uint32_t)acc;
-    (void)hi;
-}
-
-template <uint32_t K0, uint32_t K1>
-PF_INL void tmulk_5_4(const uint32_t* x, const uint32_t* y, const uint32_t* k, uint32_t* r) {
-    uint64_t acc = acc_const<K0, K1>();
-    uint32_t hi = 0u;
-    col96_1(acc, hi, x[0], y[0]);
-    r[0] = (uint32_t)acc;
-    { const uint64_t t = (uint64_t)hi + k[2]; acc = (acc >> 32) | (t << 32); hi = (uint32_t)(t >> 32); }
-    col96_2(acc, hi, x[0], x[1], y[1], y[0]);
-    r[1] = (uint32_t)acc;
-    { const uint64_t t = (uint64_t)hi + k[3]; acc = (acc >> 32) | (t << 32); hi = (uint32_t)(t >> 32); }
-    col96_3(acc, hi, x[0], x[1], x[2], y[2], y[1], y[0]);
-    r[2] = (uint32_t)acc;
-    { const uint64_t t = (uint64_t)hi + k[4]; acc = (acc >> 32) | (t << 32); hi = (uint32_t)(t >> 32); }
+}
+
+PF_INL void tmul_4_4(const uint32_t* x, const uint32_t* y, uint32_t* r) {
+    uint64_t acc = 0;
+    uint32_t hi;
+    col96_1(acc, hi, x[0], y[0]);
+    r[0] = (uint32_t)acc;
+    acc = (acc >> 32) | ((uint64_t)hi << 32);
+    col96_2(acc, hi, x[0], x[1], y[1], y[0]);
+    r[1] = (uint32_t)acc;
+    acc = (acc >> 32) | ((uint64_t)hi << 32);
+    col64_3(acc, x[0], x[1], x[2], y[2], y[1], y[0]);
+    r[2] = (uint32_t)acc;
+    acc >>= 32;
     col64_4(acc, x[0], x[1], x[2], x[3], y[3], y[2], y[1], y[0]);
     r[3] = (uint32_t)acc;
+}
+
+template <uint32_t K0, uint32_t K1, uint32_t K2, uint32_t K3, uint32_t K4>
+PF_INL void tmulk_5_4(const uint32_t* x, const uint32_t* y, uint32_t* r) {
+    uint64_t acc = acc_const<K0, K1>();
+    uint32_t hi;
+    col96_1(acc, hi, x[0], y[0]);
+    r[0] = (uint32_t)acc;
+    static_assert(K2 <= 0xFFFFFFFFu - 1u, "addend limb + 1 carries must fit 32 bits");
+    hi += K2;
+    acc = (acc >> 32) | ((uint64_t)hi << 32);
+    col96_2(acc, hi, x[0], x[1], y[1], y[0]);
+    r[1] = (uint32_t)acc;
+    static_assert(K3 <= 0xFFFFFFFFu - 2u, "addend limb + 2 carries must fit 32 bits");
+    hi += K3;
+    acc = (acc >> 32) | ((uint64_t)hi << 32);
+    col96_3(acc, hi, x[0], x[1], x[2], y[2], y[1], y[0]);
+    r[2] = (uint32_t)acc;
+    static_assert(K4 <= 0xFFFFFFFFu - 3u, "addend limb + 3 carries must fit 32 bits");
+    hi += K4;
+    acc = (acc >> 32) | ((uint64_t)hi << 32);
+    col64_4(acc, x[0], x[1], x[2], x[3], y[3], y[2], y[1], y[0]);
+    r[3] = (uint32_t)acc;
     acc >>= 32;
     col64_4(acc, x[1], x[2], x[3], x[4], y[3], y[2], y[1], y[0]);
     r[4] = (uint32_t)acc;
-    (void)hi;
-}
-
-template <uint32_t K0, uint32_t K1>
-PF_INL void tmulk_5_5(const uint32_t* x, const uint32_t* y, const uint32_t* k, uint32_t* r) {
-    uint64_t acc = acc_const<K0, K1>();
-    uint32_t hi = 0u;
-    col96_1(acc, hi, x[0], y[0]);
-    r[0] = (uint32_t)acc;
-    { const uint64_t t = (uint64_t)hi + k[2]; acc = (acc >> 32) | (t << 32); hi = (uint32_t)(t >> 32); }
-    col96_2(acc, hi, x[0], x[1], y[1], y[0]);
-    r[1] = (uint32_t)acc;
-    { const uint64_t t = (uint64_t)hi + k[3]; acc = (acc >> 32) | (t << 32); hi = (uint32_t)(t >> 32); }
-    col96_3(acc, hi, x[0], x[1], x[2], y[2], y[1], y[0]);
-    r[2] = (uint32_t)acc;
-    { const uint64_t t = (uint64_t)hi + k[4]; acc = (acc >> 32) | (t << 32); hi = (uint32_t)(t >> 32); }
+}
+
+PF_INL void tmul_5_4(const uint32_t* x, const uint32_t* y, uint32_t* r) {
+    uint64_t acc = 0;
+    uint32_t hi;
+    col96_1(acc, hi, x[0], y[0]);
+    r[0] = (uint32_t)acc;
+    acc = (acc >> 32) | ((uint64_t)hi << 32);
+    col96_2(acc, hi, x[0], x[1], y[1], y[0]);
+    r[1] = (uint32_t)acc;
+    acc = (acc >> 32) | ((uint64_t)hi << 32);
+    col96_3(acc, hi, x[0], x[1], x[2], y[2], y[1], y[0]);
+    r[2] = (uint32_t)acc;
+    acc = (acc >> 32) | ((uint64_t)hi << 32);
     col64_4(acc, x[0], x[1], x[2], x[3], y[3], y[2], y[1], y[0]);
     r[3] = (uint32_t)acc;
     acc >>= 32;
+    col64_4(acc, x[1], x[2], x[3], x[4], y[3], y[2], y[1], y[0]);
+    r[4] = (uint32_t)acc;
+}
+
+template <uint32_t K0, uint32_t K1, uint32_t K2, uint32_t K3, uint32_t K4>
+PF_INL void tmulk_5_5(const uint32_t* x, const uint32_t* y, uint32_t* r) {
+    uint64_t acc = acc_const<K0, K1>();
+    uint32_t hi;
+    col96_1(acc, hi, x[0], y[0]);
+    r[0] = (uint32_t)acc;
+    static_assert(K2 <= 0xFFFFFFFFu - 1u, "addend limb + 1 carries must fit 32 bits");
+    hi += K2;
+    acc = (acc >> 32) | ((uint64_t)hi << 32);
+    col96_2(acc, hi, x[0], x[1], y[1], y[0]);
+    r[1] = (uint32_t)acc;
+    static_assert(K3 <= 0xFFFFFFFFu - 2u, "addend limb + 2 carries must fit 32 bits");
+    hi += K3;
+    acc = (acc >> 32) | ((uint64_t)hi << 32);
+    col96_3(acc, hi, x[0], x[1], x[2], y[2], y[1], y[0]);
+    r[2] = (uint32_t)acc;
+    static_assert(K4 <= 0xFFFFFFFFu - 3u, "addend limb + 3 carries must fit 32 bits");
+    hi += K4;
+    acc = (acc >> 32) | ((uint64_t)hi << 32);
+    col64_4(acc, x[0], x[1], x[2], x[3], y[3], y[2], y[1], y[0]);
+    r[3] = (uint32_t)acc;
+    acc >>= 32;
     col64_5(acc, x[0], x[1], x[2], x[3], x[4], y[4], y[3], y[2], y[1], y[0]);
     r[4] = (uint32_t)acc;
-    (void)hi;
-}
-
-template <uint32_t K0, uint32_t K1>
-PF_INL void tmulk_6_5(const uint32_t* x, const uint32_t* y, const uint32_t* k, uint32_t* r) {
-    uint64_t acc = acc_const<K0, K1>();
-    uint32_t hi = 0u;
-    col96_1(acc, hi, x[0], y[0]);
-    r[0] = (uint32_t)acc;
-    { const uint64_t t = (uint64_t)hi + k[2]; acc = (acc >> 32) | (t << 32); hi = (uint32_t)(t >> 32); }
-    col96_2(acc, hi, x[0], x[1], y[1], y[0]);
-    r[1] = (uint32_t)acc;
-    { const uint64_t t = (uint64_t)hi + k[3]; acc = (acc >> 32) | (t << 32); hi = (uint32_t)(t >> 32); }
-    col96_3(acc, hi, x[0], x[1], x[2], y[2], y[1], y[0]);
-    r[2] = (uint32_t)acc;
-    { const uint64_t t = (uint64_t)hi + k[4]; acc = (acc >> 32) | (t << 32); hi = (uint32_t)(t >> 32); }
+}
+
+PF_INL void tmul_5_5(const uint32_t* x, const uint32_t* y, uint32_t* r) {
+    uint64_t acc = 0;
+    uint32_t hi;
+    col96_1(acc, hi, x[0], y[0]);
+    r[0] = (uint32_t)acc;
+    acc = (acc >> 32) | ((uint64_t)hi << 32);
+    col96_2(acc, hi, x[0], x[1], y[1], y[0]);
+    r[1] = (uint32_t)acc;
+    acc = (acc >> 32) | ((uint64_t)hi << 32);
+    col96_3(acc, hi, x[0], x[1], x[2], y[2], y[1], y[0]);
+    r[2] = (uint32_t)acc;
+    acc = (acc >> 32) | ((uint64_t)hi << 32);
+    col64_4(acc, x[0], x[1], x[2], x[3], y[3], y[2], y[1], y[0]);
+    r[3] = (uint32_t)acc;
+    acc >>= 32;
+    col64_5(acc, x[0], x[1], x[2], x[3], x[4], y[4], y[3], y[2], y[1], y[0]);
+    r[4] = (uint32_t)acc;
+}
+
+template <uint32_t K0, uint32_t K1, uint32_t K2, uint32_t K3, uint32_t K4, uint32_t K5>
+PF_INL void tmulk_6_5(const uint32_t* x, const uint32_t* y, uint32_t* r) {
+    uint64_t acc = acc_const<K0, K1>();
+    uint32_t hi;
+    col96_1(acc, hi, x[0], y[0]);
+    r[0] = (uint32_t)acc;
+    static_assert(K2 <= 0xFFFFFFFFu - 1u, "addend limb + 1 carries must fit 32 bits");
+    hi += K2;
+    acc = (acc >> 32) | ((uint64_t)hi << 32);
+    col96_2(acc, hi, x[0], x[1], y[1], y[0]);
+    r[1] = (uint32_t)acc;
+    static_assert(K3 <= 0xFFFFFFFFu - 2u, "addend limb + 2 carries must fit 32 bits");
+    hi += K3;
+    acc = (acc >> 32) | ((uint64_t)hi << 32);
+    col96_3(acc, hi, x[0], x[1], x[2], y[2], y[1], y[0]);
+    r[2] = (uint32_t)acc;
+    static_assert(K4 <= 0xFFFFFFFFu - 3u, "addend limb + 3 carries must fit 32 bits");
+    hi += K4;
+    acc = (acc >> 32) | ((uint64_t)hi << 32);
     col96_4(acc, hi, x[0], x[1], x[2], x[3], y[3], y[2], y[1], y[0]);
     r[3] = (uint32_t)acc;
-    { const uint64_t t = (uint64_t)hi + k[5]; acc = (acc >> 32) | (t << 32); hi = (uint32_t)(t >> 32); }
+    static_assert(K5 <= 0xFFFFFFFFu - 4u, "addend limb + 4 carries must fit 32 bits");
+    hi += K5;
+    acc = (acc >> 32) | ((uint64_t)hi << 32);
     col64_5(acc, x[0], x[1], x[2], x[3], x[4], y[4], y[3], y[2], y[1], y[0]);
     r[4] = (uint32_t)acc;
     acc >>= 32;
     col64_5(acc, x[1], x[2], x[3], x[4], x[5], y[4], y[3], y[2], y[1], y[0]);
     r[5] = (uint32_t)acc;
-    (void)hi;
-}
-
-template <uint32_t K0, uint32_t K1>
-PF_INL void tmulk_6_6(const uint32_t* x, const uint32_t* y, const uint32_t* k, uint32_t* r) {
-    uint64_t acc = acc_const<K0, K1>();
-    uint32_t hi = 0u;
-    col96_1(acc, hi, x[0], y[0]);
-    r[0] = (uint32_t)acc;
-    { const uint64_t t = (uint64_t)hi + k[2]; acc = (acc >> 32) | (t << 32); hi = (uint32_t)(t >> 32); }
-    col96_2(acc, hi, x[0], x[1], y[1], y[0]);
-    r[1] = (uint32_t)acc;
-    { const uint64_t t = (uint64_t)hi + k[3]; acc = (acc >> 32) | (t << 32); hi = (uint32_t)(t >> 32); }
-    col96_3(acc, hi, x[0], x[1], x[2], y[2], y[1], y[0]);
-    r[2] = (uint32_t)acc;
-    { const uint64_t t = (uint64_t)hi + k[4]; acc = (acc >> 32) | (t << 32); hi = (uint32_t)(t >> 32); }
+}
+
+PF_INL void tmul_6_5(const uint32_t* x, const uint32_t* y, uint32_t* r) {
+    uint64_t acc = 0;
+    uint32_t hi;
+    col96_1(acc, hi, x[0], y[0]);
+    r[0] = (uint32_t)acc;
+    acc = (acc >> 32) | ((uint64_t)hi << 32);
+    col96_2(acc, hi, x[0], x[1], y[1], y[0]);
+    r[1] = (uint32_t)acc;
+    acc = (acc >> 32) | ((uint64_t)hi << 32);
+    col96_3(acc, hi, x[0], x[1], x[2], y[2], y[1], y[0]);
+    r[2] = (uint32_t)acc;
+    acc = (acc >> 32) | ((uint64_t)hi << 32);
     col96_4(acc, hi, x[0], x[1], x[2], x[3], y[3], y[2], y[1], y[0]);
     r[3] = (uint32_t)acc;
-    { const uint64_t t = (uint64_t)hi + k[5]; acc = (acc >> 32) | (t << 32); hi = (uint32_t)(t >> 32); }
+    acc = (acc >> 32) | ((uint64_t)hi << 32);
+    col64_5(acc, x[0], x[1], x[2], x[3], x[4], y[4], y[3], y[2], y[1], y[0]);
+    r[4] = (uint32_t)acc;
+    acc >>= 32;
+    col64_5(acc, x[1], x[2], x[3], x[4], x[5], y[4], y[3], y[2], y[1], y[0]);
+    r[5] = (uint32_t)acc;
+}
+
+template <uint32_t K0, uint32_t K1, uint32_t K2, uint32_t K3, uint32_t K4, uint32_t K5>
+PF_INL void tmulk_6_6(const uint32_t* x, const uint32_t* y, uint32_t* r) {
+    uint64_t acc = acc_const<K0, K1>();
+    uint32_t hi;
+    col96_1(acc, hi, x[0], y[0]);
+    r[0] = (uint32_t)acc;
+    static_assert(K2 <= 0xFFFFFFFFu - 1u, "addend limb + 1 carries must fit 32 bits");
+    hi += K2;
+    acc = (acc >> 32) | ((uint64_t)hi << 32);
+    col96_2(acc, hi, x[0], x[1], y[1], y[0]);
+    r[1] = (uint32_t)acc;
+    static_assert(K3 <= 0xFFFFFFFFu - 2u, "addend limb + 2 carries must fit 32 bits");
+    hi += K3;
+    acc = (acc >> 32) | ((uint64_t)hi << 32);
+    col96_3(acc, hi, x[0], x[1], x[2], y[2], y[1], y[0]);
+    r[2] = (uint32_t)acc;
+    static_assert(K4 <= 0xFFFFFFFFu - 3u, "addend limb + 3 carries must fit 32 bits");
+    hi += K4;
+    acc = (acc >> 32) | ((uint64_t)hi << 32);
+    col96_4(acc, hi, x[0], x[1], x[2], x[3], y[3], y[2], y[1], y[0]);
+    r[3] = (uint32_t)acc;
+    static_assert(K5 <= 0xFFFFFFFFu - 4u, "addend limb + 4 carries must fit 32 bits");
+    hi += K5;
+    acc = (acc >> 32) | ((uint64_t)hi << 32);
     col64_5(acc, x[0], x[1], x[2], x[3], x[4], y[4], y[3], y[2], y[1], y[0]);
     r[4] = (uint32_t)acc;
     acc >>= 32;
     col64_6(acc, x[0], x[1], x[2], x[3], x[4], x[5], y[5], y[4], y[3], y[2], y[1], y[0]);
     r[5] = (uint32_t)acc;
-    (void)hi;
-}
-
-template <uint32_t K0, uint32_t K1>
-PF_INL void tmulk_7_6(const uint32_t* x, const uint32_t* y, const uint32_t* k, uint32_t* r) {
-    uint64_t acc = acc_const<K0, K1>();
-    uint32_t hi = 0u;
-    col96_1(acc, hi, x[0], y[0]);
-    r[0] = (uint32_t)acc;
-    { const uint64_t t = (uint64_t)hi + k[2]; acc = (acc >> 32) | (t << 32); hi = (uint32_t)(t >> 32); }
-    col96_2(acc, hi, x[0], x[1], y[1], y[0]);
-    r[1] = (uint32_t)acc;
-    { const uint64_t t = (uint64_t)hi + k[3]; acc = (acc >> 32) | (t << 32); hi = (uint32_t)(t >> 32); }
-    col96_3(acc, hi, x[0], x[1], x[2], y[2], y[1], y[0]);
-    r[2] = (uint32_t)acc;
-    { const uint64_t t = (uint64_t)hi + k[4]; acc = (acc >> 32) | (t << 32); hi = (uint32_t)(t >> 32); }
+}
+
+PF_INL void tmul_6_6(const uint32_t* x, const uint32_t* y, uint32_t* r) {
+    uint64_t acc = 0;
+    uint32_t hi;
+    col96_1(acc, hi, x[0], y[0]);
+    r[0] = (uint32_t)acc;
+    acc = (acc >> 32) | ((uint64_t)hi << 32);
+    col96_2(acc, hi, x[0], x[1], y[1], y[0]);
+    r[1] = (uint32_t)acc;
+    acc = (acc >> 32) | ((uint64_t)hi << 32);
+    col96_3(acc, hi, x[0], x[1], x[2], y[2], y[1], y[0]);
+    r[2] = (uint32_t)acc;
+    acc = (acc >> 32) | ((uint64_t)hi << 32);
     col96_4(acc, hi, x[0], x[1], x[2], x[3], y[3], y[2], y[1], y[0]);
     r[3] = (uint32_t)acc;
-    { const uint64_t t = (uint64_t)hi + k[5]; acc = (acc >> 32) | (t << 32); hi = (uint32_t)(t >> 32); }
-    col96_5(acc, hi, x[0], x[1], x[2], x[3], x[4], y[4], y[3], y[2], y[1], y[0]);
-    r[4] = (uint32_t)acc;
-    { const uint64_t t = (uint64_t)hi + k[6]; acc = (acc >> 32) | (t << 32); hi = (uint32_t)(t >> 32); }
+    acc = (acc >> 32) | ((uint64_t)hi << 32);
+    col64_5(acc, x[0], x[1], x[2], x[3], x[4], y[4], y[3], y[2], y[1], y[0]);
+    r[4] = (uint32_t)acc;
+    acc >>= 32;
     col64_6(acc, x[0], x[1], x[2], x[3], x[4], x[5], y[5], y[4], y[3], y[2], y[1], y[0]);
     r[5] = (uint32_t)acc;
+}
+
+template <uint32_t K0, uint32_t K1, uint32_t K2, uint32_t K3, uint32_t K4, uint32_t K5, uint32_t K6>
+PF_INL void tmulk_7_6(const uint32_t* x, const uint32_t* y, uint32_t* r) {
+    uint64_t acc = acc_const<K0, K1>();
+    uint32_t hi;
+    col96_1(acc, hi, x[0], y[0]);
+    r[0] = (uint32_t)acc;
+    static_assert(K2 <= 0xFFFFFFFFu - 1u, "addend limb + 1 carries must fit 32 bits");
+    hi += K2;
+    acc = (acc >> 32) | ((uint64_t)hi << 32);
+    col96_2(acc, hi, x[0], x[1], y[1], y[0]);
+    r[1] = (uint32_t)acc;
+    static_assert(K3 <= 0xFFFFFFFFu - 2u, "addend limb + 2 carries must fit 32 bits");
+    hi += K3;
+    acc = (acc >> 32) | ((uint64_t)hi << 32);
+    col96_3(acc, hi, x[0], x[1], x[2], y[2], y[1], y[0]);
+    r[2] = (uint32_t)acc;
+    static_assert(K4 <= 0xFFFFFFFFu - 3u, "addend limb + 3 carries must fit 32 bits");
+    hi += K4;
+    acc = (acc >> 32) | ((uint64_t)hi << 32);
+    col96_4(acc, hi, x[0], x[1], x[2], x[3], y[3], y[2], y[1], y[0]);
+    r[3] = (uint32_t)acc;
+    static_assert(K5 <= 0xFFFFFFFFu - 4u, "addend limb + 4 carries must fit 32 bits");
+    hi += K5;
+    acc = (acc >> 32) | ((uint64_t)hi << 32);
+    col96_5(acc, hi, x[0], x[1], x[2], x[3], x[4], y[4], y[3], y[2], y[1], y[0]);
+    r[4] = (uint32_t)acc;
+    static_assert(K6 <= 0xFFFFFFFFu - 5u, "addend limb + 5 carries must fit 32 bits");
+    hi += K6;
+    acc = (acc >> 32) | ((uint64_t)hi << 32);
+    col64_6(acc, x[0], x[1], x[2], x[3], x[4], x[5], y[5], y[4], y[3], y[2], y[1], y[0]);
+    r[5] = (uint32_t)acc;
     acc >>= 32;
     col64_6(acc, x[1], x[2], x[3], x[4], x[5], x[6], y[5], y[4], y[3], y[2], y[1], y[0]);
     r[6] = (uint32_t)acc;
-    (void)hi;
-}
-
-template <uint32_t K0, uint32_t K1>
-PF_INL void tmulk_7_7(const uint32_t* x, const uint32_t* y, const uint32_t* k, uint32_t* r) {
-    uint64_t acc = acc_const<K0, K1>();
-    uint32_t hi = 0u;
-    col96_1(acc, hi, x[0], y[0]);
-    r[0] = (uint32_t)acc;
-    { const uint64_t t = (uint64_t)hi + k[2]; acc = (acc >> 32) | (t << 32); hi = (uint32_t)(t >> 32); }
-    col96_2(acc, hi, x[0], x[1], y[1], y[0]);
-    r[1] = (uint32_t)acc;
-    { const uint64_t t = (uint64_t)hi + k[3]; acc = (acc >> 32) | (t << 32); hi = (uint32_t)(t >> 32); }
-    col96_3(acc, hi, x[0], x[1], x[2], y[2], y[1], y[0]);
-    r[2] = (uint32_t)acc;
-    { const uint64_t t = (uint64_t)hi + k[4]; acc = (acc >> 32) | (t << 32); hi = (uint32_t)(t >> 32); }
+}
+
+PF_INL void tmul_7_6(const uint32_t* x, const uint32_t* y, uint32_t* r) {
+    uint64_t acc = 0;
+    uint32_t hi;
+    col96_1(acc, hi, x[0], y[0]);
+    r[0] = (uint32_t)acc;
+    acc = (acc >> 32) | ((uint64_t)hi << 32);
+    col96_2(acc, hi, x[0], x[1], y[1], y[0]);
+    r[1] = (uint32_t)acc;
+    acc = (acc >> 32) | ((uint64_t)hi << 32);
+    col96_3(acc, hi, x[0], x[1], x[2], y[2], y[1], y[0]);
+    r[2] = (uint32_t)acc;
+    acc = (acc >> 32) | ((uint64_t)hi << 32);
     col96_4(acc, hi, x[0], x[1], x[2], x[3], y[3], y[2], y[1], y[0]);
     r[3] = (uint32_t)acc;
-    { const uint64_t t = (uint64_t)hi + k[5]; acc = (acc >> 32) | (t << 32); hi = (uint32_t)(t >> 32); }
+    acc = (acc >> 32) | ((uint64_t)hi << 32);
     col96_5(acc, hi, x[0], x[1], x[2], x[3], x[4], y[4], y[3], y[2], y[1], y[0]);
     r[4] = (uint32_t)acc;
-    { const uint64_t t = (uint64_t)hi + k[6]; acc = (acc >> 32) | (t << 32); hi = (uint32_t)(t >> 32); }
+    acc = (acc >> 32) | ((uint64_t)hi << 32);
     col64_6(acc, x[0], x[1], x[2], x[3], x[4], x[5], y[5], y[4], y[3], y[2], y[1], y[0]);
     r[5] = (uint32_t)acc;
     acc >>= 32;
+    col64_6(acc, x[1], x[2], x[3], x[4], x[5], x[6], y[5], y[4], y[3], y[2], y[1], y[0]);
+    r[6] = (uint32_t)acc;
+}
+
+template <uint32_t K0, uint32_t K1, uint32_t K2, uint32_t K3, uint32_t K4, uint32_t K5, uint32_t K6>
+PF_INL void tmulk_7_7(const uint32_t* x, const uint32_t* y, uint32_t* r) {
+    uint64_t acc = acc_const<K0, K1>();
+    uint32_t hi;
+    col96_1(acc, hi, x[0], y[0]);
+    r[0] = (uint32_t)acc;
+    static_assert(K2 <= 0xFFFFFFFFu - 1u, "addend limb + 1 carries must fit 32 bits");
+    hi += K2;
+    acc = (acc >> 32) | ((uint64_t)hi << 32);
+    col96_2(acc, hi, x[0], x[1], y[1], y[0]);
+    r[1] = (uint32_t)acc;
+    static_assert(K3 <= 0xFFFFFFFFu - 2u, "addend limb + 2 carries must fit 32 bits");
+    hi += K3;
+    acc = (acc >> 32) | ((uint64_t)hi << 32);
+    col96_3(acc, hi, x[0], x[1], x[2], y[2], y[1], y[0]);
+    r[2] = (uint32_t)acc;
+    static_assert(K4 <= 0xFFFFFFFFu - 3u, "addend limb + 3 carries must fit 32 bits");
+    hi += K4;
+    acc = (acc >> 32) | ((uint64_t)hi << 32);
+    col96_4(acc, hi, x[0], x[1], x[2], x[3], y[3], y[2], y[1], y[0]);
+    r[3] = (uint32_t)acc;
+    static_assert(K5 <= 0xFFFFFFFFu - 4u, "addend limb + 4 carries must fit 32 bits");
+    hi += K5;
+    acc = (acc >> 32) | ((uint64_t)hi << 32);
+    col96_5(acc, hi, x[0], x[1], x[2], x[3], x[4], y[4], y[3], y[2], y[1], y[0]);
+    r[4] = (uint32_t)acc;
+    static_assert(K6 <= 0xFFFFFFFFu - 5u, "addend limb + 5 carries must fit 32 bits");
+    hi += K6;
+    acc = (acc >> 32) | ((uint64_t)hi << 32);
+    col64_6(acc, x[0], x[1], x[2], x[3], x[4], x[5], y[5], y[4], y[3], y[2], y[1], y[0]);
+    r[5] = (uint32_t)acc;
+    acc >>= 32;
     col64_7(acc, x[0], x[1], x[2], x[3], x[4], x[5], x[6], y[6], y[5], y[4], y[3], y[2], y[1], y[0]);
     r[6] = (uint32_t)acc;
-    (void)hi;
-}
-
-template <int L, int LY, uint32_t K0, uint32_t K1>
-PF_INL void tmulk(const uint32_t* x, const uint32_t* y, const uint32_t* k, uint32_t* r) {
+}
+
+PF_INL void tmul_7_7(const uint32_t* x, const uint32_t* y, uint32_t* r) {
+    uint64_t acc = 0;
+    uint32_t hi;
+    col96_1(acc, hi, x[0], y[0]);
+    r[0] = (uint32_t)acc;
+    acc = (acc >> 32) | ((uint64_t)hi << 32);
+    col96_2(acc, hi, x[0], x[1], y[1], y[0]);
+    r[1] = (uint32_t)acc;
+    acc = (acc >> 32) | ((uint64_t)hi << 32);
+    col96_3(acc, hi, x[0], x[1], x[2], y[2], y[1], y[0]);
+    r[2] = (uint32_t)acc;
+    acc = (acc >> 32) | ((uint64_t)hi << 32);
+    col96_4(acc, hi, x[0], x[1], x[2], x[3], y[3], y[2], y[1], y[0]);
+    r[3] = (uint32_t)acc;
+    acc = (acc >> 32) | ((uint64_t)hi << 32);
+    col96_5(acc, hi, x[0], x[1], x[2], x[3], x[4], y[4], y[3], y[2], y[1], y[0]);
+    r[4] = (uint32_t)acc;
+    acc = (acc >> 32) | ((uint64_t)hi << 32);
+    col64_6(acc, x[0], x[1], x[2], x[3], x[4], x[5], y[5], y[4], y[3], y[2], y[1], y[0]);
+    r[5] = (uint32_t)acc;
+    acc >>= 32;
+    col64_7(acc, x[0], x[1], x[2], x[3], x[4], x[5], x[6], y[6], y[5], y[4], y[3], y[2], y[1], y[0]);
+    r[6] = (uint32_t)acc;
+}
+
+template <int L, int LY, uint32_t K0, uint32_t K1, uint32_t K2, uint32_t K3, uint32_t K4, uint32_t K5, uint32_t K6>
+PF_INL void tmulk(const uint32_t* x, const uint32_t* y, uint32_t* r) {
     static_assert(L >= 1 && L <= 7 && (LY == L || LY == L - 1) && LY >= 1, "shape");
-    if constexpr (L == 1 && LY == 1) tmulk_1_1<K0, K1>(x, y, k, r);
-    if constexpr (L == 2 && LY == 1) tmulk_2_1<K0, K1>(x, y, k, r);
-    if constexpr (L == 2 && LY == 2) tmulk_2_2<K0, K1>(x, y, k, r);
-    if constexpr (L == 3 && LY == 2) tmulk_3_2<K0, K1>(x, y, k, r);
-    if constexpr (L == 3 && LY == 3) tmulk_3_3<K0, K1>(x, y, k, r);
-    if constexpr (L == 4 && LY == 3) tmulk_4_3<K0, K1>(x, y, k, r);
-    if constexpr (L == 4 && LY == 4) tmulk_4_4<K0, K1>(x, y, k, r);
-    if constexpr (L == 5 && LY == 4) tmulk_5_4<K0, K1>(x, y, k, r);
-    if constexpr (L == 5 && LY == 5) tmulk_5_5<K0, K1>(x, y, k, r);
-    if constexpr (L == 6 && LY == 5) tmulk_6_5<K0, K1>(x, y, k, r);
-    if constexpr (L == 6 && LY == 6) tmulk_6_6<K0, K1>(x, y, k, r);
-    if constexpr (L == 7 && LY == 6) tmulk_7_6<K0, K1>(x, y, k, r);
-    if constexpr (L == 7 && LY == 7) tmulk_7_7<K0, K1>(x, y, k, r);
-}
-
-}
+    constexpr bool ZERO = (K0 | K1 | K2 | K3 | K4 | K5 | K6) == 0u;
+    if constexpr (L == 1 && LY == 1 && ZERO) tmul_1_1(x, y, r);
+    if constexpr (L == 1 && LY == 1 && !ZERO) tmulk_1_1<K0>(x, y, r);
+    if constexpr (L == 2 && LY == 1 && ZERO) tmul_2_1(x, y, r);
+    if constexpr (L == 2 && LY == 1 && !ZERO) tmulk_2_1<K0, K1>(x, y, r);
+    if constexpr (L == 2 && LY == 2 && ZERO) tmul_2_2(x, y, r);
+    if constexpr (L == 2 && LY == 2 && !ZERO) tmulk_2_2<K0, K1>(x, y, r);
+    if constexpr (L == 3 && LY == 2 && ZERO) tmul_3_2(x, y, r);
+    if constexpr (L == 3 && LY == 2 && !ZERO) tmulk_3_2<K0, K1, K2>(x, y, r);
+    if constexpr (L == 3 && LY == 3 && ZERO) tmul_3_3(x, y, r);
+    if constexpr (L == 3 && LY == 3 && !ZERO) tmulk_3_3<K0, K1, K2>(x, y, r);
+    if constexpr (L == 4 && LY == 3 && ZERO) tmul_4_3(x, y, r);
+    if constexpr (L == 4 && LY == 3 && !ZERO) tmulk_4_3<K0, K1, K2, K3>(x, y, r);
+    if constexpr (L == 4 && LY == 4 && ZERO) tmul_4_4(x, y, r);
+    if constexpr (L == 4 && LY == 4 && !ZERO) tmulk_4_4<K0, K1, K2, K3>(x, y, r);
+    if constexpr (L == 5 && LY == 4 && ZERO) tmul_5_4(x, y, r);
+    if constexpr (L == 5 && LY == 4 && !ZERO) tmulk_5_4<K0, K1, K2, K3, K4>(x, y, r);
+    if constexpr (L == 5 && LY == 5 && ZERO) tmul_5_5(x, y, r);
+    if constexpr (L == 5 && LY == 5 && !ZERO) tmulk_5_5<K0, K1, K2, K3, K4>(x, y, r);
+    if constexpr (L == 6 && LY == 5 && ZERO) tmul_6_5(x, y, r);
+    if constexpr (L == 6 && LY == 5 && !ZERO) tmulk_6_5<K0, K1, K2, K3, K4, K5>(x, y, r);
+    if constexpr (L == 6 && LY == 6 && ZERO) tmul_6_6(x, y, r);
+    if constexpr (L == 6 && LY == 6 && !ZERO) tmulk_6_6<K0, K1, K2, K3, K4, K5>(x, y, r);
+    if constexpr (L == 7 && LY == 6 && ZERO) tmul_7_6(x, y, r);
+    if constexpr (L == 7 && LY == 6 && !ZERO) tmulk_7_6<K0, K1, K2, K3, K4, K5, K6>(x, y, r);
+    if constexpr (L == 7 && LY == 7 && ZERO) tmul_7_7(x, y, r);
+    if constexpr (L == 7 && LY == 7 && !ZERO) tmulk_7_7<K0, K1, K2, K3, K4, K5, K6>(x, y, r);
+}
+
+}
```
